# nl1xx/simple-multimodal

Hardware: AMD Instinct MI355X
Metric: fusion fwd+bwd samples/sec at B=16 d=768 (higher is better)
Workload: dtype bf16

## Files before the change

include/mmfusion.h:

```cpp
#ifndef MMFUSION_H
#define MMFUSION_H

#include <stddef.h>
#include <stdint.h>

#ifdef __cplusplus
extern "C" {
#endif

#define MMF_ABI_VERSION 1

enum {
  MMF_OK = 0,
  MMF_E_SHAPE = -1,
  MMF_E_DTYPE = -2,
  MMF_E_ALIGN = -3,
  MMF_E_LAUNCH = -4,
  MMF_E_UNSUPPORTED = -5
};

int mmf_version(void);
const char* mmf_last_error(void);
int mmf_device_cu_count(void);

#define MMF_GEMM_MAX_PROBLEMS 48
enum { MMF_GEMM_NT = 0, MMF_GEMM_NN = 1, MMF_GEMM_TN = 2 };
enum {
  MMF_EPI_BIAS = 1,
  MMF_EPI_RELU = 2,
  MMF_EPI_MASK_AUX = 4,
  MMF_EPI_ADD_AUX = 8,
  MMF_EPI_ACCUM = 16,
  MMF_EPI_COLSUM_A = 32,
  MMF_EPI_DROPOUT = 64
};

typedef struct mmf_gemm_problem {
  const void* A;
  const void* B;
  void* C;
  const float* bias;
  const void* aux;
  int32_t M, N, K;
  int32_t lda, ldb, ldc, ldaux;
} mmf_gemm_problem;

int mmf_gemm_grouped(const mmf_gemm_problem* problems, int num_problems, int layout,
                     int epilogue, int out_f32, void* stream);
typedef struct mmf_gemm_extra {
  float alpha;
  float dropout_p;
  const uint64_t* rng_state;
  uint32_t site;
} mmf_gemm_extra;
int mmf_gemm_grouped_ex(const mmf_gemm_problem* problems, int num_problems, int layout, int epilogue,
                        int out_f32, const mmf_gemm_extra* extra, void* stream);

int mmf_gemm_select_impl(int impl);
int mmf_gemm_last_impl(void);
int mmf_gemm_set_persistent_workgroups(int n);

#define MMF_SKINNY_MAX_PROBLEMS 24
typedef struct mmf_skinny_problem {
  const void* X;
  const void* W;
  void* Y;
  const float* bias;
  const void* aux;
  int32_t M, N, K;
  int32_t ldx, ldw, ldy, ldaux;
} mmf_skinny_problem;
int mmf_skinny_linear_fwd(const mmf_skinny_problem* problems, int num_problems, int flags, int out_f32, void* stream);
int mmf_skinny_linear_dgrad(const mmf_skinny_problem* problems, int num_problems, int flags, float alpha, int out_f32,
                            void* stream);
int mmf_skinny_last_strip(void);
typedef struct mmf_skinny_problem_ex {
  mmf_skinny_problem p;
  void* Y2;
  const void* gate;
  void* dz;
  int32_t ldy2, ldgate, lddz, reserved;
} mmf_skinny_problem_ex;
typedef struct mmf_skinny_extra {
  int32_t x_f32;
  int32_t gate_f32;
  float gate_scale;
  float dropout_p;
  const uint64_t* rng_state;
  uint32_t site;
  uint32_t reserved;
} mmf_skinny_extra;
int mmf_skinny_linear_fwd_ex(const mmf_skinny_problem_ex* problems, int num_problems, int flags, int out_f32,
                             const mmf_skinny_extra* extra, void* stream);
int mmf_skinny_linear_dgrad_ex(const mmf_skinny_problem_ex* problems, int num_problems, int flags, float alpha, int out_f32,
                               const mmf_skinny_extra* extra, void* stream);

int mmf_fusion_loss(const float* logits, int ldl, const int64_t* targets, int B, int C, float label_smoothing,
                    const float* const* extra, const float* extra_w, int n_extra, float* loss, float* dlogits, void* stream);
int mmf_modality_dropout(const float* const* x, float* const* y, float* keep, int B, int d, float p,
                         const uint64_t* rng_state, uint32_t site, int draw, void* stream);

int mmf_distill_kl(const float* student, int lds, const float* teacher, int ldt, int B, int C, float temperature,
                   float* loss, float* dstudent, void* stream);
int mmf_fusion_loss_kd(const float* logits, int ldl, const int64_t* targets, int B, int C, float label_smoothing,
                       const float* const* extra, const float* extra_w, int n_extra,
                       const float* teacher, int ldt, float temperature, float kd_weight,
                       float* loss, float* dlogits, void* stream);

int mmf_robust_head_fwd(const float* const f[3], const float* h, const float* W2, const float* b2,
                        const float* const Wm[3], const float* const bm[3], int avail, float* a, float* const p[3],
                        float* wn, float* y, int B, int d, int C, void* stream);
int mmf_robust_head_bwd(const float* const f[3], const float* h, const float* W2, const float* const Wm[3],
                        const float* a, const float* const p[3], const float* wn, int avail, const float* g,
                        const float* const dP[3], const float* dA, const float* dN, float* const df[3], float* dh,
                        float* dW2, float* db2, float* const dWm[3], float* const dbm[3], int B, int d, int C, void* stream);

int mmf_fewshot_proto_fwd(const float* const s[3], float* sf, float* mean, int n_way, int n_shot, int d, void* stream);
int mmf_fewshot_proto_bwd(const float* dmean, const float* dsf, float* ds, int n_way, int n_shot, int d, void* stream);
int mmf_fewshot_dist_fwd(const float* const q[3], const float* P, float* qf, float* dist, float* pred, int Nq, int n_way,
                         int d, void* stream);
int mmf_fewshot_dist_bwd(const float* qf, const float* P, const float* dist, const float* pred, const float* gdist,
                         const float* gpred, float* dq, float* dp, int Nq, int n_way, int d, void* stream);

#define MMF_EVAL_MAX_HEADS 4
#define MMF_EVAL_NSUMS 4
int mmf_eval_accumulate(const float* const* logits, const int* ld, int n_heads, const int64_t* targets, int B, int C,
                        float label_smoothing, int64_t* counts, double* sums, int64_t* pred_out, int64_t* target_out,
                        float* prob_out, int64_t row0, int64_t capacity, void* stream);

#define MMF_ATTN_MAX_PROBLEMS 12
typedef struct mmf_attn_problem {
  const void* Q; const void* K; const void* V;
  void* O;
  float* LSE;
  const void* dO;
  float* delta;
  void* dQ; void* dK; void* dV;
  int32_t B, H, Tq, Tk;
  int32_t ldq, ldk, ldv, ldo;
} mmf_attn_problem;

int mmf_attn_fwd_grouped(const mmf_attn_problem* problems, int num_problems, int head_dim,
                         float scale, void* stream);
int mmf_attn_bwd_grouped(const mmf_attn_problem* problems, int num_problems, int head_dim,
                         float scale, void* stream);
int mmf_attn_fwd_grouped_ex(const mmf_attn_problem* problems, int num_problems, int head_dim, float scale,
                            float dropout_p, const uint64_t* rng_state, uint32_t site, void* stream);
int mmf_attn_select_impl(int impl);
int mmf_attn_bwd_grouped_ex(const mmf_attn_problem* problems, int num_problems, int head_dim, float scale,
                            float dropout_p, const uint64_t* rng_state, uint32_t site, void* stream);

#define MMF_LN_MAX_PROBLEMS 8
typedef struct mmf_ln_problem {
  const void* x;
  void* y;
  const float* gamma;
  const float* beta;
  float* mean;
  float* rstd;
  const void* dy;
  void* dx;
  float* dgamma;
  float* dbeta;
  int32_t rows;
} mmf_ln_problem;

int mmf_layernorm_fwd_grouped(const mmf_ln_problem* problems, int num_problems, int d, float eps,
                              void* stream);
size_t mmf_layernorm_bwd_workspace_bytes(int d);
int mmf_layernorm_bwd_grouped(const mmf_ln_problem* problems, int num_problems, int d,
                              void* workspace, size_t workspace_bytes, void* stream);
int mmf_layernorm_last_form(void);

int mmf_cast_f32_to_bf16(const float* src, void* dst, int64_t n, void* stream);
int mmf_cast_bf16_to_f32(const void* src, float* dst, int64_t n, void* stream);
int mmf_cast_f32_to_bf16_2d(const float* src, void* dst, int rows, int cols, int ld_src, void* stream);
int mmf_cast_bf16_to_f32_scaled(const void* src, float* dst, int64_t n, float scale, void* stream);
int mmf_add3_bf16(const void* a, const void* b, const void* c, void* y, int64_t n, void* stream);
#define MMF_ADD3_MAX 8
typedef struct mmf_add3_problem {
  const void* a; const void* b; const void* c;
  void* y;
  int64_t n;
} mmf_add3_problem;
int mmf_add3_grouped(const mmf_add3_problem* problems, int num_problems, void* stream);
#define MMF_ADDN_MAX 8
int mmf_addn_bf16(const void* const* xs, int n, void* y, int64_t numel, int out_f32, void* stream);
#define MMF_ADDN_GROUP_MAX 4
typedef struct mmf_addn_problem {
  const void* x[MMF_ADDN_MAX];
  void* y;
  int64_t numel;
  int32_t n;
} mmf_addn_problem;
int mmf_addn_grouped(const mmf_addn_problem* problems, int num_problems, void* stream);
int mmf_meanpool_fwd(const void* x, void* y, int B, int T, int d, int ldy, void* stream);
int mmf_meanpool_bwd(const void* dy, void* dx, int B, int T, int d, int lddy, void* stream);
#define MMF_POOL_MAX 4
int mmf_meanpool_cat_fwd(const void* const* xs, const int* Ts, int n, void* y, int B, int d, int ldy, void* stream);
int mmf_meanpool_cat_bwd(const void* dy, void* const* dxs, const int* Ts, int n, int B, int d, int lddy, void* stream);
int mmf_colsum_bf16(const void* x, float* out, int M, int N, int ldx, void* stream);
#define MMF_COLSUM_MAX_PROBLEMS 24
typedef struct mmf_colsum_problem {
  const void* x;
  float* out;
  int32_t M, N, ldx;
} mmf_colsum_problem;
int mmf_colsum_grouped(const mmf_colsum_problem* problems, int num_problems, void* stream);
int mmf_dropout(const void* x, void* y, int64_t n, int is_f32, float p, const uint64_t* rng_state,
                uint32_t site, void* stream);
#define MMF_ZERO_MAX_RANGES 48
int mmf_zero_ranges_f32(float* base, const int64_t* starts, const int64_t* ends, int n, void* stream);
int mmf_relu_bwd_bf16(const void* dy, const void* y, void* dx, int64_t n, void* stream);
int mmf_relu_bwd_mixed(const void* dy, int dy_f32, const void* y, int y_f32, void* dx, int64_t n, void* stream);

typedef struct mmf_gat3_params {
  int32_t B, heads, C, relu;
  float negative_slope, dropout_p;
  const uint64_t* rng_state;
  uint32_t site;
} mmf_gat3_params;
int mmf_gat3_dense_fwd(const float* h, const float* att_src, const float* att_dst, const float* bias,
                       void* y_bf16, void* pooled_bf16, float* alpha, float* sdots,
                       const mmf_gat3_params* p, void* stream);
int mmf_gat3_dense_bwd(const float* h, const float* att_src, const float* att_dst, const void* y_bf16,
                       const float* alpha, const float* sdots, const void* dy_bf16, const void* dpooled_bf16,
                       float* dh, float* datt_src, float* datt_dst, float* dbias,
                       const mmf_gat3_params* p, void* stream);
int mmf_infonce_fwd(const float* const z[3], float* const n[3], float* inv_norm, float* losses, float* lse,
                    int B, int D, float temperature, void* stream);
int mmf_infonce_bwd(const float* const n[3], const float* inv_norm, const float* lse, const float* const dn[3],
                    const float* const dloss[3], float* const dz[3], int B, int D, float temperature, void* stream);
int mmf_adaptive_combine_fwd(const float* hp, const float* W2, const float* b2, const float* attended,
                             float* aw, void* weighted_bf16, int B, int d, void* stream);
int mmf_adaptive_combine_bwd(const float* hp, const float* W2, const float* attended, const float* aw,
                             const void* dweighted_bf16, const float* daw, float* dattended, float* dhp,
                             float* dW2, float* db2, int B, int d, void* stream);
int mmf_adaptive_attn_weights(const void* qkv_bf16, float* w, int B, int heads, int head_dim, void* stream);
int mmf_attn_weights_mean(const void* qkv_bf16, float* w, int B, int T, int heads, int head_dim, void* stream);
int mmf_linear_narrow_fwd(const float* x, const float* W, const float* b, float* y, int M, int N, int K, void* stream);
int mmf_linear_narrow_bwd(const float* x, const float* W, const float* dy, float* dx, float* dW, float* db,
                          int M, int N, int K, void* stream);
int mmf_stack3_embed_fwd(const float* f0, const float* f1, const float* f2, const float* emb, void* x_bf16,
                         int B, int d, int ldf, void* stream);
int mmf_stack3_embed_bwd(const void* dx_bf16, float* d0, float* d1, float* d2, float* demb, int B, int d, int ldd,
                         void* stream);
int mmf_rowmask_apply(const float* x, const float* mask, float* y, int B, int d, void* stream);

int mmf_sqnorm_f32(const float* x, int64_t n, float* out, void* stream);
int mmf_adamw_advance(int64_t* step, float* hparams, const double* sched, void* stream);
int mmf_adamw_step(float* master, const float* grad, float* exp_avg, float* exp_avg_sq, void* shadow_bf16,
                   int64_t n, const float* hparams, const float* gnorm_sq, void* stream);

int mmf_gemm_f32_grouped(const mmf_gemm_problem* problems, int num_problems, int layout, int epilogue, float alpha,
                         void* stream);
int mmf_gemm_f32_batched(const mmf_gemm_problem* problem, int layout, int epilogue, float alpha, int nb0, int nb1,
                         const int64_t strideA[2], const int64_t strideB[2], const int64_t strideC[2], void* stream);
int mmf_softmax_rows_f32(float* S, int64_t rows, int cols, float scale, void* stream);
int mmf_softmax_bwd_rows_f32(const float* P, float* dP, int64_t rows, int cols, float scale, void* stream);
int mmf_layernorm_f32_fwd(const float* x, float* y, const float* gamma, const float* beta, float* mean, float* rstd,
                          int rows, int d, float eps, void* stream);
int mmf_layernorm_f32_bwd(const float* x, const float* dy, const float* gamma, const float* mean, const float* rstd,
                          float* dx, float* dgamma, float* dbeta, int rows, int d, void* stream);

typedef struct mmf_bilstm_args {
  const void* gx;
  const void* w_hh[2];
  const float* b_ih[2];
  const float* b_hh[2];
  void* y;
  float* gates;
  float* cell;
  const void* dy;
  void* dgates;
  int32_t T, B, H;
} mmf_bilstm_args;
size_t mmf_bilstm_workspace_bytes(void);
int mmf_bilstm_layer_fwd(const mmf_bilstm_args* args, void* workspace, size_t workspace_bytes, void* stream);
int mmf_bilstm_layer_bwd(const mmf_bilstm_args* args, void* workspace, size_t workspace_bytes, void* stream);

int mmf_swap01(const void* in, void* out, int n0, int n1, int d, int in_f32, int out_f32, void* stream);

#ifdef __cplusplus
}
#endif
#endif
```

simple-multimodal_amd/csrc/gemm6.hip:

```cpp
#include "gemm6_parts.h"


#ifndef MMF_G6_DBG
#define MMF_G6_DBG 0
#endif

namespace {

template <bool A_KR, bool B_KR, int BK, int NS, bool OUT_F32>
__device__ __forceinline__ void gemm6_body(const GemmArgs& args, const int total_tiles, char* smem) {
  constexpr int TILE = 256 * BK * 2, STAGE = 2 * TILE, NG = BK / 16, PPO = BK / 8, PPW = 2 * PPO;
  constexpr int WA = A_KR ? 256 : BK, WB = B_KR ? 256 : BK;
  static_assert(NG == 2 || NG == 4, "BK is 32 or 64");

  const int bid = mmf_xcd_tile(blockIdx.x, total_tiles, args.xcd_granule);
  int pi = 0;
  while (pi + 1 < args.nprob && bid >= args.tile_start[pi + 1]) ++pi;
  const mmf_gemm_problem& P = args.p[pi];
  int m0, n0;
  tile_origin(P, bid - args.tile_start[pi], m0, n0);

  const int tid = threadIdx.x, lane = tid & 63;
  const int wave = __builtin_amdgcn_readfirstlane(tid >> 6);
  const int wm = wave >> 1, wn = wave & 1;
  const int M = P.M, N = P.N, K = P.K;
  const int KT = (K + BK - 1) / BK;

  unsigned voff[PPW];
#pragma unroll
  for (int i = 0; i < PPO; ++i) {
    voff[i] = piece_voff<A_KR, BK>(wave + 4 * i, P.lda, lane);
    voff[PPO + i] = piece_voff<B_KR, BK>(wave + 4 * i, P.ldb, lane);
  }
  const unsigned short* Ab = static_cast<const unsigned short*>(P.A) + (A_KR ? (size_t)m0 : (size_t)m0 * P.lda);
  const unsigned short* Bb = static_cast<const unsigned short*>(P.B) + (B_KR ? (size_t)n0 : (size_t)n0 * P.ldb);
  const long recA = A_KR ? ((long)(K - 1) * P.lda + (M - m0)) * 2 : ((long)(M - m0 - 1) * P.lda + K) * 2;
  const long recB = B_KR ? ((long)(K - 1) * P.ldb + (N - n0)) * 2 : ((long)(N - n0 - 1) * P.ldb + K) * 2;
  const int kstepA = A_KR ? BK * P.lda : BK, kstepB = B_KR ? BK * P.ldb : BK;
  char* const my_pieces = smem + wave * 1024;

  auto issue_piece = [&](int kt, int i, bool empty = false) {
    char* st = my_pieces + (kt % NS) * STAGE;
    if (i < PPO) {
      const __amdgpu_buffer_rsrc_t rs = __builtin_amdgcn_make_buffer_rsrc(
          const_cast<unsigned short*>(Ab + (size_t)kt * kstepA), 0, empty ? 0 : (int)(recA - (long)kt * kstepA * 2), 0x00020000);
      __builtin_amdgcn_raw_ptr_buffer_load_lds(rs, (lds_void_t*)(st + i * 4096), 16, voff[i], 0, 0, 0);
    } else {
      const __amdgpu_buffer_rsrc_t rs = __builtin_amdgcn_make_buffer_rsrc(
          const_cast<unsigned short*>(Bb + (size_t)kt * kstepB), 0, empty ? 0 : (int)(recB - (long)kt * kstepB * 2), 0x00020000);
      __builtin_amdgcn_raw_ptr_buffer_load_lds(rs, (lds_void_t*)(st + TILE + (i - PPO) * 4096), 16, voff[i], 0, 0, 0);
    }
  };

  typedef int i32x4_t __attribute__((ext_vector_type(4)));
  auto mkdesc = [](const unsigned short* p, long rec) {
    const unsigned long long a = (unsigned long long)(uintptr_t)p;
    return i32x4_t{(int)(unsigned)a, (int)((unsigned)(a >> 32) & 0xffffu), (int)rec, 0x00020000};
  };
  auto advance = [](i32x4_t& d, int bytes) {
    const unsigned long long a = (((unsigned long long)(unsigned)d[1] << 32) | (unsigned)d[0]) + (unsigned long long)bytes;
    d[0] = (int)(unsigned)a; d[1] = (int)(unsigned)(a >> 32); d[2] -= bytes;
  };
  i32x4_t dA = mkdesc(Ab + (size_t)(NS - 1) * kstepA, recA - (long)(NS - 1) * kstepA * 2);
  i32x4_t dB = mkdesc(Bb + (size_t)(NS - 1) * kstepB, recB - (long)(NS - 1) * kstepB * 2);
  const unsigned lds_pieces = (unsigned)(uintptr_t)(const __attribute__((address_space(3))) char*)my_pieces;
  auto hot_piece = [&](auto ic, const unsigned ring_base) {
    constexpr int I = decltype(ic)::value, OFF = I < PPO ? I * 4096 : TILE + (I - PPO) * 4096;
    if constexpr (MMF_G6_DBG & 16) {
      asm volatile("s_nop 0\n\ts_nop 0\n\ts_nop 0" ::: "memory");
      __builtin_amdgcn_sched_barrier(0);
      return;
    }
    if (I < PPO) asm volatile("s_add_i32 m0, %0, %3\n\ts_nop 0\n\tbuffer_load_dwordx4 %1, %2, 0 offen lds" ::"s"(ring_base), "v"(voff[I]), "s"(dA), "n"(OFF) : "memory");
    else         asm volatile("s_add_i32 m0, %0, %3\n\ts_nop 0\n\tbuffer_load_dwordx4 %1, %2, 0 offen lds" ::"s"(ring_base), "v"(voff[I]), "s"(dB), "n"(OFF) : "memory");
    __builtin_amdgcn_sched_barrier(0);
  };

  unsigned la0, la1, lb0, lb1;
  Frag4<A_KR>::lane_parts(WA, lane, la0, la1);
  Frag4<B_KR>::lane_parts(WB, lane, lb0, lb1);
  const unsigned smem_base = (unsigned)(uintptr_t)(const __attribute__((address_space(3))) char*)smem;
  const unsigned qa = (unsigned)(A_KR ? 512 * 4 * wm : (WA / 32) * 2048 * 4 * wm);
  const unsigned qb = (unsigned)(B_KR ? 512 * 4 * wn : (WB / 32) * 2048 * 4 * wn);
  la0 += smem_base + qa; la1 += smem_base + qa;
  lb0 += smem_base + TILE + qb; lb1 += smem_base + TILE + qb;

  f32x16_t acc[4][4];
  const bool do_colsum = A_KR && (args.epi & MMF_EPI_COLSUM_A) && n0 == 0;
  const bool edge_m = m0 + BM > M;
  bool colok[4];
#pragma unroll
  for (int j = 0; j < 4; ++j) colok[j] = m0 + 128 * wm + 32 * j + (lane & 31) < M;
  f32x16_t csum;
#pragma unroll
  for (int e = 0; e < 16; ++e) csum[e] = 0.f;
  u32x4_t sel[4];
#pragma unroll
  for (int j = 0; j < 4; ++j) {
    const unsigned w = ((lane & 31) == j) ? 0x3f803f80u : 0u;
    sel[j] = u32x4_t{w, w, w, w};
  }

#pragma unroll
  for (int s = 0; s < NS; ++s)
    if (s < KT) {
#pragma unroll
      for (int i = 0; i < PPW; ++i) issue_piece(s, i);
    }
  if (KT >= NS) vm_wait<PPW * (NS - 1)>(); else vm_wait<0>();
  __builtin_amdgcn_s_barrier();
  Frag4<A_KR> fa[2];
  Frag4<B_KR> fb[2];
  fa[0].template issue<WA, 0, 0>(la0, la1);
  fb[0].template issue<WB, 0, 0>(lb0, lb1);
  frag_wait(fa[0], fb[0]);

  auto mf = [&](const Frag4<A_KR>& a, const Frag4<B_KR>& b, int i, bool first = false) {
    const int tm = i >> 2, tn = i & 3;
    const f32x16_t zero = {0.f, 0.f, 0.f, 0.f, 0.f, 0.f, 0.f, 0.f, 0.f, 0.f, 0.f, 0.f, 0.f, 0.f, 0.f, 0.f};
    acc[tn][tm] = __builtin_amdgcn_mfma_f32_32x32x16_bf16(b.get(tn), a.get(tm), first ? zero : acc[tn][tm], 0, 0, 0);
    if (A_KR && do_colsum && tn == 3 && (tm >> 1) == wn) {
      u32x4_t fm = __builtin_bit_cast(u32x4_t, a.get(tm));
      if (edge_m && !colok[tm]) fm = u32x4_t{0u, 0u, 0u, 0u};
      asm volatile("s_nop 1\n\tv_mfma_f32_32x32x16_bf16 %0, %1, %2, %0" : "+v"(csum) : "v"(sel[tm]), "v"(fm));
    }
    __builtin_amdgcn_sched_barrier(0);
  };
#define MMF_G6_READ(dstA, dstB, G, u, so)                                                              \
  do {                                                                                                 \
    if ((u) == 0) dstA.template issue1<WA, G, 0, 0>(la0 + (so), la1 + (so));                            \
    if ((u) == 1) dstA.template issue1<WA, G, 0, 1>(la0 + (so), la1 + (so));                            \
    if ((u) == 2) dstA.template issue1<WA, G, 0, 2>(la0 + (so), la1 + (so));                            \
    if ((u) == 3) dstA.template issue1<WA, G, 0, 3>(la0 + (so), la1 + (so));                            \
    if ((u) == 4) dstB.template issue1<WB, G, 0, 0>(lb0 + (so), lb1 + (so));                            \
    if ((u) == 5) dstB.template issue1<WB, G, 0, 1>(lb0 + (so), lb1 + (so));                            \
    if ((u) == 6) dstB.template issue1<WB, G, 0, 2>(lb0 + (so), lb1 + (so));                            \
    if ((u) == 7) dstB.template issue1<WB, G, 0, 3>(lb0 + (so), lb1 + (so));                            \
    __builtin_amdgcn_sched_barrier(0);                                                                 \
  } while (0)
  static_assert(PPW == 4 + 4 * (NG - 1), "four late pieces + four per not-last substep");
#define MMF_G6_SUBSTEP(cur, nxt, G)                                                                    \
  do {                                                                                                 \
    _Pragma("unroll") for (int i = 0; i < 16; ++i) {                                                   \
      mf(fa[cur], fb[cur], i, FIRST && (G) == 1);                                                      \
      if (i < 8 && !(MMF_G6_DBG & 4)) MMF_G6_READ(fa[nxt], fb[nxt], G, i, so);                        \
      if (i == 8 && !(MMF_G6_DBG & 1)) { if (early) hot_piece(std::integral_constant<int, 4 * (G)>{}, ring_prev); }      \
      if (i == 10 && !(MMF_G6_DBG & 1)) { if (early) hot_piece(std::integral_constant<int, 4 * (G) + 1>{}, ring_prev); } \
      if (i == 12 && !(MMF_G6_DBG & 1)) { if (early) hot_piece(std::integral_constant<int, 4 * (G) + 2>{}, ring_prev); } \
      if (i == 14 && !(MMF_G6_DBG & 1)) { if (early) hot_piece(std::integral_constant<int, 4 * (G) + 3>{}, ring_prev); } \
    }                                                                                                  \
    if (!(MMF_G6_DBG & 4)) frag_wait(fa[nxt], fb[nxt]);                                                \
  } while (0)

  using T = std::true_type;
  using F = std::false_type;
  auto stage = [&](auto next_c, auto steady_c, auto first_c, const int kt, const int ahead, const bool e, const bool l) {
    constexpr bool NEXT = decltype(next_c)::value, STEADY = decltype(steady_c)::value, FIRST = decltype(first_c)::value;
    const bool early = STEADY || e, late = STEADY || l;
    const unsigned so = (unsigned)((kt % NS) * STAGE);
    const unsigned ring_cur = lds_pieces + so, ring_prev = lds_pieces + (unsigned)(((kt + NS - 1) % NS) * STAGE);
    if constexpr (NG == 4) {
      MMF_G6_SUBSTEP(0, 1, 1);
      MMF_G6_SUBSTEP(1, 0, 2);
      MMF_G6_SUBSTEP(0, 1, 3);
    } else {
      MMF_G6_SUBSTEP(0, 1, 1);
    }
    const unsigned sn = (unsigned)(((kt + 1) % NS) * STAGE);
#pragma unroll
    for (int i = 0; i < 4; ++i) mf(fa[1], fb[1], i);
    if constexpr (NEXT) {
      if constexpr (!(MMF_G6_DBG & 2)) {
        if constexpr (STEADY) {
          vm_wait<PPW * (NS - 2)>();
        } else {
          if (ahead >= 3) vm_wait<PPW * 3>(); else if (ahead == 2) vm_wait<PPW * 2>(); else if (ahead == 1) vm_wait<PPW>(); else vm_wait<0>();
        }
        __builtin_amdgcn_s_barrier();
      }
      if constexpr (!(MMF_G6_DBG & 32)) {
        advance(dA, kstepA * 2);
        advance(dB, kstepB * 2);
      }
    }
    __builtin_amdgcn_sched_barrier(0);
#pragma unroll
    for (int i = 4; i < 16; ++i) {
      mf(fa[1], fb[1], i);
      if constexpr (NEXT && !(MMF_G6_DBG & 4)) { if (i < 12) MMF_G6_READ(fa[0], fb[0], 0, i - 4, sn); }
      if (i == 12 && !(MMF_G6_DBG & 1)) { if (late) hot_piece(std::integral_constant<int, 0>{}, ring_cur); }
      if (i == 13 && !(MMF_G6_DBG & 1)) { if (late) hot_piece(std::integral_constant<int, 1>{}, ring_cur); }
      if (i == 14 && !(MMF_G6_DBG & 1)) { if (late) hot_piece(std::integral_constant<int, 2>{}, ring_cur); }
      if (i == 15 && !(MMF_G6_DBG & 1)) { if (late) hot_piece(std::integral_constant<int, 3>{}, ring_cur); }
    }
    if constexpr (NEXT && !(MMF_G6_DBG & 4)) frag_wait(fa[0], fb[0]);
  };
  {
    int kt = 0;
    if (KT > 1) {
      stage(T{}, F{}, T{}, 0, min(NS - 2, KT - 2), false, NS < KT);
      for (kt = 1; kt + NS < KT; ++kt) stage(T{}, T{}, F{}, kt, NS - 2, true, true);
      for (; kt + 1 < KT; ++kt) stage(T{}, F{}, F{}, kt, min(NS - 2, KT - 2 - kt), kt - 1 + NS < KT, kt + NS < KT);
      stage(F{}, F{}, F{}, kt, 0, false, false);
    } else {
      stage(F{}, F{}, T{}, 0, 0, false, false);
    }
  }
#undef MMF_G6_SUBSTEP
#undef MMF_G6_READ

  if (A_KR && do_colsum) {
    asm volatile("s_nop 15\n\ts_nop 7" : "+v"(csum));
    if (lane < 32) {
#pragma unroll
      for (int tm = 0; tm < 4; ++tm) {
        const int m = m0 + 128 * wm + 32 * tm + lane;
        if ((tm >> 1) == wn && m < M) atomicAdd(const_cast<float*>(P.bias) + m, csum[tm]);
      }
    }
  }
  if constexpr (MMF_G6_DBG & 64) {
    float keep = 0.f;
#pragma unroll
    for (int i = 0; i < 4; ++i)
#pragma unroll
      for (int j = 0; j < 4; ++j) keep += acc[i][j][0];
    if (keep == 12345.678f) static_cast<float*>(P.C)[lane] = keep;
    return;
  }
  tile_epilogue<OUT_F32>(args, P, pi, m0 + 128 * wm, n0 + 128 * wn, acc, lane, args.epi);
}

template <bool A_KR, bool B_KR, int BK, int NS, bool OUT_F32>
__global__ __launch_bounds__(NTHREADS, 1)
void gemm6_grouped_kernel(const GemmArgs args, const int total_tiles) {
  __shared__ __attribute__((aligned(1024))) char smem[NS * 2 * 256 * BK * 2];
  gemm6_body<A_KR, B_KR, BK, NS, OUT_F32>(args, total_tiles, smem);
}

template <bool A_KR, bool B_KR, int BK, int NS>
void launch(const GemmArgs& a, int total, int out_f32, hipStream_t s) {
  if (out_f32) hipLaunchKernelGGL((gemm6_grouped_kernel<A_KR, B_KR, BK, NS, true>), dim3(total), dim3(NTHREADS), 0, s, a, total);
  else         hipLaunchKernelGGL((gemm6_grouped_kernel<A_KR, B_KR, BK, NS, false>), dim3(total), dim3(NTHREADS), 0, s, a, total);
}
}

bool mmf_gemm6_supports(const mmf_gemm_problem* problems, int num_problems, int layout) {
  if (layout == MMF_GEMM_TN) return true;
  const int bk = 32;
  for (int i = 0; i < num_problems; ++i)
    if (problems[i].K % bk) return false;
  return true;
}
bool mmf_gemm6_supports_epi(int epilogue, int out_f32) { return !(out_f32 && (epilogue & (MMF_EPI_MASK_AUX | MMF_EPI_ADD_AUX))); }

int mmf_gemm6_launch(const mmf_gemm_problem* problems, int num_problems, int layout, int epilogue,
                     int out_f32, const mmf_gemm_extra* extra, hipStream_t s) {
  GemmArgs a;
  a.nprob = num_problems;
  a.epi = epilogue;
  a.xcd_granule = mmf_xcd_granule();
  a.alpha = extra ? extra->alpha : 1.f;
  a.drop_thresh = extra ? mmf_drop_thresh(extra->dropout_p) : 0u;
  a.site = extra ? extra->site : 0u;
  a.rng_state = extra ? reinterpret_cast<const unsigned long long*>(extra->rng_state) : nullptr;
  int total = 0;
  for (int i = 0; i < num_problems; ++i) {
    const mmf_gemm_problem& p = problems[i];
    const size_t a_bytes = (size_t)(layout == MMF_GEMM_TN ? p.K : p.M) * p.lda * 2;
    const size_t b_bytes = (size_t)(layout == MMF_GEMM_NT ? p.N : p.K) * p.ldb * 2;
    if (a_bytes >= 0x7fffffffull || b_bytes >= 0x7fffffffull)
      MMF_FAIL(MMF_E_UNSUPPORTED, "mmf_gemm_grouped[%d]: operand larger than 2 GiB", i);
    if (layout != MMF_GEMM_TN && p.K % 32)
      MMF_FAIL(MMF_E_UNSUPPORTED, "mmf_gemm_grouped[%d]: the one-wave-per-SIMD kernel needs K %% 32 == 0 for NT / NN (K = %d)", i, p.K);
    if (out_f32 && (epilogue & (MMF_EPI_MASK_AUX | MMF_EPI_ADD_AUX)))
      MMF_FAIL(MMF_E_UNSUPPORTED, "mmf_gemm_grouped: the one-wave-per-SIMD kernel has no aux epilogue with f32 output");
    a.tile_start[i] = total;
    total += ((p.M + BM - 1) / BM) * ((p.N + BN - 1) / BN);
    a.p[i] = p;
  }
  a.tile_start[num_problems] = total;
  static const int cfg = [] { const char* e = getenv("MMF_GEMM6_CFG"); return e ? atoi(e) : 0; }();
  bool k64 = true;
  for (int i = 0; i < num_problems; ++i) k64 = k64 && (problems[i].K % 64 == 0 || layout == MMF_GEMM_TN);
  const int c = (cfg == 2 && !k64) ? 0 : cfg;
  switch (layout) {
    case MMF_GEMM_NT:
      if (c == 1) launch<false, false, 32, 5>(a, total, out_f32, s); else if (c == 2) launch<false, false, 64, 2>(a, total, out_f32, s);
      else launch<false, false, 32, 4>(a, total, out_f32, s);
      break;
    case MMF_GEMM_NN:
      if (c == 1) launch<false, true, 32, 5>(a, total, out_f32, s); else if (c == 2) launch<false, true, 64, 2>(a, total, out_f32, s);
      else launch<false, true, 32, 4>(a, total, out_f32, s);
      break;
    default:
      if (c == 1) launch<true, true, 32, 5>(a, total, out_f32, s); else if (c == 2) launch<true, true, 64, 2>(a, total, out_f32, s);
      else launch<true, true, 32, 4>(a, total, out_f32, s);
      break;
  }
  MMF_CHECK_LAUNCH("mmf_gemm_grouped(v6)");
  return MMF_OK;
}
```

simple-multimodal_amd/csrc/gemm6_parts.h:

```cpp
#pragma once
#include "mmf_internal.h"
#include "lds_image.h"
#include <stdlib.h>
#include <type_traits>

namespace {

constexpr int BM = 256, BN = 256;
constexpr int NTHREADS = 256;

struct GemmArgs {
  int nprob;
  int epi;
  int xcd_granule;
  float alpha;
  unsigned drop_thresh, site;
  const unsigned long long* rng_state;
  int tile_start[MMF_GEMM_MAX_PROBLEMS + 1];
  short orig[MMF_GEMM_MAX_PROBLEMS];
  mmf_gemm_problem p[MMF_GEMM_MAX_PROBLEMS];
};

typedef __attribute__((address_space(3))) void lds_void_t;

template <int N> __device__ __forceinline__ void vm_wait() { asm volatile("s_waitcnt vmcnt(%0)" ::"n"(N) : "memory"); }

template <int OFF>
__device__ __forceinline__ u32x4_t lds_read_b128(unsigned addr) {
  u32x4_t r;
  asm volatile("ds_read_b128 %0, %1 offset:%2" : "=v"(r) : "v"(addr), "n"(OFF));
  return r;
}
template <int OFF>
__device__ __forceinline__ u32x2_t lds_read_tr(unsigned addr) {
  u32x2_t r;
  asm volatile("ds_read_b64_tr_b16 %0, %1 offset:%2" : "=v"(r) : "v"(addr), "n"(OFF));
  return r;
}

template <bool KR> struct Frag4;
template <> struct Frag4<false> {
  u32x4_t v[4];
  static __device__ __forceinline__ void lane_parts(int W, int lane, unsigned& a0, unsigned& a1) {
    const int r = lane & 31, h = lane >> 5, s = (r >> 2) & 3;
    const unsigned base = (unsigned)((W / 32) * 512 * (r >> 3) + 64 * (r & 7));
    a0 = base + 16u * (unsigned)(h ^ s);
    a1 = base + 16u * (unsigned)((2 + h) ^ s);
  }
  template <int W, int G, int D0>
  __device__ __forceinline__ void issue(unsigned t0, unsigned t1) {
    const unsigned t = (G & 1) ? t1 : t0;
    constexpr int S = (W / 32) * 2048;
    v[0] = lds_read_b128<S * (D0 + 0) + 512 * (G >> 1)>(t);
    v[1] = lds_read_b128<S * (D0 + 1) + 512 * (G >> 1)>(t);
    v[2] = lds_read_b128<S * (D0 + 2) + 512 * (G >> 1)>(t);
    v[3] = lds_read_b128<S * (D0 + 3) + 512 * (G >> 1)>(t);
  }
  template <int W, int G, int D0, int I>
  __device__ __forceinline__ void issue1(unsigned t0, unsigned t1) {
    v[I] = lds_read_b128<(W / 32) * 2048 * (D0 + I) + 512 * (G >> 1)>((G & 1) ? t1 : t0);
  }
  __device__ __forceinline__ bf16x8_t get(int i) const { return __builtin_bit_cast(bf16x8_t, v[i]); }
};
template <> struct Frag4<true> {
  u32x2_t lo[4], hi[4];
  static __device__ __forceinline__ void lane_parts(int, int lane, unsigned& a0, unsigned& a1) {
    const int h = lane >> 5, g = (lane >> 4) & 1, q = (lane >> 2) & 3, p = lane & 3;
    const unsigned c = (unsigned)(2 * g + (p >> 1));
    a0 = (unsigned)(4096 * h + 64 * q) + 16u * (c ^ (unsigned)(2 * h)) + 8u * (unsigned)(p & 1);
    a1 = (unsigned)(4096 * h + 64 * (4 + q)) + 16u * (c ^ (unsigned)(2 * h + 1)) + 8u * (unsigned)(p & 1);
  }
  template <int W, int G, int D0>
  __device__ __forceinline__ void issue(unsigned t0, unsigned t1) {
    lo[0] = lds_read_tr<8192 * G + 512 * (D0 + 0)>(t0); hi[0] = lds_read_tr<8192 * G + 512 * (D0 + 0)>(t1);
    lo[1] = lds_read_tr<8192 * G + 512 * (D0 + 1)>(t0); hi[1] = lds_read_tr<8192 * G + 512 * (D0 + 1)>(t1);
    lo[2] = lds_read_tr<8192 * G + 512 * (D0 + 2)>(t0); hi[2] = lds_read_tr<8192 * G + 512 * (D0 + 2)>(t1);
    lo[3] = lds_read_tr<8192 * G + 512 * (D0 + 3)>(t0); hi[3] = lds_read_tr<8192 * G + 512 * (D0 + 3)>(t1);
  }
  template <int W, int G, int D0, int I>
  __device__ __forceinline__ void issue1(unsigned t0, unsigned t1) {
    lo[I] = lds_read_tr<8192 * G + 512 * (D0 + I)>(t0); hi[I] = lds_read_tr<8192 * G + 512 * (D0 + I)>(t1);
  }
  __device__ __forceinline__ bf16x8_t get(int i) const {
    const u32x4_t w = {lo[i][0], lo[i][1], hi[i][0], hi[i][1]};
    return __builtin_bit_cast(bf16x8_t, w);
  }
};
__device__ __forceinline__ void frag_wait(Frag4<false>& a, Frag4<false>& b) {
  asm volatile("s_waitcnt lgkmcnt(0)" : "+v"(a.v[0]), "+v"(a.v[1]), "+v"(a.v[2]), "+v"(a.v[3]), "+v"(b.v[0]), "+v"(b.v[1]), "+v"(b.v[2]), "+v"(b.v[3]));
}
__device__ __forceinline__ void frag_wait(Frag4<false>& a, Frag4<true>& b) {
  asm volatile("s_waitcnt lgkmcnt(0)" : "+v"(a.v[0]), "+v"(a.v[1]), "+v"(a.v[2]), "+v"(a.v[3]), "+v"(b.lo[0]), "+v"(b.lo[1]), "+v"(b.lo[2]), "+v"(b.lo[3]),
               "+v"(b.hi[0]), "+v"(b.hi[1]), "+v"(b.hi[2]), "+v"(b.hi[3]));
}
__device__ __forceinline__ void frag_wait(Frag4<true>& a, Frag4<true>& b) {
  asm volatile("s_waitcnt lgkmcnt(0)" : "+v"(a.lo[0]), "+v"(a.lo[1]), "+v"(a.lo[2]), "+v"(a.lo[3]), "+v"(a.hi[0]), "+v"(a.hi[1]), "+v"(a.hi[2]), "+v"(a.hi[3]),
               "+v"(b.lo[0]), "+v"(b.lo[1]), "+v"(b.lo[2]), "+v"(b.lo[3]), "+v"(b.hi[0]), "+v"(b.hi[1]), "+v"(b.hi[2]), "+v"(b.hi[3]));
}

template <bool KR, int BK>
__device__ __forceinline__ unsigned piece_voff(int p, int ld, int lane) {
  constexpr int NC = (KR ? 256 : BK) / 32;
  const int st = 2 * p + (lane >> 5), rg = st / NC, cc = st % NC;
  const int w = lane & 31, row = 8 * rg + (w >> 2), ch = 4 * cc + ((w & 3) ^ ((row >> 2) & 3));
  return (unsigned)(row * ld * 2 + ch * 16);
}

__device__ __forceinline__ void tile_origin(const mmf_gemm_problem& P, const int t, int& m0, int& n0) {
  const int tiles_m = (P.M + BM - 1) / BM, tiles_n = (P.N + BN - 1) / BN;
#ifdef MMF_GEMM_GROUPM
  constexpr int GROUP_M = MMF_GEMM_GROUPM;
#else
  constexpr int GROUP_M = 8;
#endif
  const int grp = t / (GROUP_M * tiles_n), rem = t % (GROUP_M * tiles_n);
  const int gm = min(GROUP_M, tiles_m - grp * GROUP_M);
  m0 = (grp * GROUP_M + rem % gm) * BM;
  n0 = (rem / gm) * BN;
}

template <bool OUT_F32, int CT>
__device__ __forceinline__ void tile_epilogue_mode(const GemmArgs& args, const mmf_gemm_problem& P, const int pi, const int mb, const int nb,
                                                   f32x16_t (&acc)[4][4], const int lane, const int epi_all) {
  constexpr int MODE = CT < 0 ? 3 : 0;
  const int M = P.M, N = P.N;
  const int epi = CT < 0 ? epi_all : (CT | (epi_all & MMF_EPI_ACCUM));
  const unsigned short* __restrict__ aux = static_cast<const unsigned short*>(P.aux);
  const bool do_drop = MODE == 3 && (epi & MMF_EPI_DROPOUT);
  const unsigned drop_key = do_drop ? mmf_rng_key(*args.rng_state, args.site, (unsigned)pi) : 0u;
  const float drop_scale = do_drop ? 1.f / (1.f - (float)args.drop_thresh * (1.f / 4294967296.f)) : 1.f;
  const float alpha = MODE == 3 ? args.alpha : 1.f;
  const bool use_aux = epi & (MMF_EPI_MASK_AUX | MMF_EPI_ADD_AUX);
  const bool use_old = OUT_F32 && (epi & MMF_EPI_ACCUM);
  const int h = lane >> 5;
  auto ncol = [&](int tn, int g) { return nb + 32 * tn + 8 * g + 4 * h; };

  f32x4_t bv[4][4];
#pragma unroll
  for (int tn = 0; tn < 4; ++tn)
#pragma unroll
    for (int g = 0; g < 4; ++g) {
      bv[tn][g] = f32x4_t{0.f, 0.f, 0.f, 0.f};
      if ((epi & MMF_EPI_BIAS) && ncol(tn, g) < N) bv[tn][g] = *reinterpret_cast<const f32x4_t*>(P.bias + ncol(tn, g));
    }
  auto finish = [&](f32x4_t v, const f32x4_t& b, const u32x2_t& a, int m, int n) -> f32x4_t {
    if constexpr (CT >= 0) {
      if constexpr (CT & MMF_EPI_BIAS) v += b;
      if constexpr (CT & MMF_EPI_RELU) {
#pragma unroll
        for (int e = 0; e < 4; ++e) v[e] = fmaxf(v[e], 0.f);
      }
      if constexpr (CT & (MMF_EPI_MASK_AUX | MMF_EPI_ADD_AUX)) {
        const float a0 = bf16lo(a[0]), a1 = bf16hi(a[0]), a2 = bf16lo(a[1]), a3 = bf16hi(a[1]);
        if constexpr (CT & MMF_EPI_MASK_AUX) {
          v[0] = a0 > 0.f ? v[0] : 0.f; v[1] = a1 > 0.f ? v[1] : 0.f;
          v[2] = a2 > 0.f ? v[2] : 0.f; v[3] = a3 > 0.f ? v[3] : 0.f;
        } else {
          v[0] += a0; v[1] += a1; v[2] += a2; v[3] += a3;
        }
      }
      return v;
    }
    v += b;
    if (epi & MMF_EPI_RELU) {
#pragma unroll
      for (int e = 0; e < 4; ++e) v[e] = fmaxf(v[e], 0.f);
    }
    if (do_drop) {
      const unsigned idx = (unsigned)m * (unsigned)N + (unsigned)n;
#pragma unroll
      for (int e = 0; e < 4; ++e) v[e] = mmf_keep(drop_key, idx + e, args.drop_thresh) ? v[e] * drop_scale : 0.f;
    }
    const float a0 = bf16lo(a[0]), a1 = bf16hi(a[0]), a2 = bf16lo(a[1]), a3 = bf16hi(a[1]);
    if (epi & MMF_EPI_MASK_AUX) {
      v[0] = a0 > 0.f ? v[0] : 0.f; v[1] = a1 > 0.f ? v[1] : 0.f;
      v[2] = a2 > 0.f ? v[2] : 0.f; v[3] = a3 > 0.f ? v[3] : 0.f;
    }
    v *= alpha;
    if (epi & MMF_EPI_ADD_AUX) { v[0] += a0; v[1] += a1; v[2] += a2; v[3] += a3; }
    return v;
  };
  const bool wide = (N & 7) == 0 && (P.ldc & 7) == 0;
  if constexpr (OUT_F32) {
    f32x4_t oldv[2][4];
    auto preload_tile = [&](int t, int slot) {
      const int tm = t >> 2, tn = t & 3, m = mb + 32 * tm + (lane & 31);
#pragma unroll
      for (int g = 0; g < 4; ++g) {
        oldv[slot][g] = f32x4_t{0.f, 0.f, 0.f, 0.f};
        if (m < M && ncol(tn, g) < N)
          oldv[slot][g] = *reinterpret_cast<const f32x4_t*>(static_cast<const float*>(P.C) + (size_t)m * P.ldc + ncol(tn, g));
      }
    };
    if (use_old) preload_tile(0, 0);
#pragma unroll
    for (int t = 0; t < 16; ++t) {
      const int tm = t >> 2, tn = t & 3, m = mb + 32 * tm + (lane & 31);
      f32x4_t v[4];
#pragma unroll
      for (int g = 0; g < 4; ++g) {
        v[g] = f32x4_t{acc[tn][tm][4 * g], acc[tn][tm][4 * g + 1], acc[tn][tm][4 * g + 2], acc[tn][tm][4 * g + 3]};
        v[g] = finish(v[g], bv[tn][g], u32x2_t{0u, 0u}, m, ncol(tn, g));
        if (use_old) v[g] += oldv[t & 1][g];
      }
      if (use_old && t + 1 < 16) preload_tile(t + 1, (t + 1) & 1);
#pragma unroll
      for (int g = 0; g < 4; ++g)
        if (m < M && ncol(tn, g) < N)
          *reinterpret_cast<f32x4_t*>(static_cast<float*>(P.C) + (size_t)m * P.ldc + ncol(tn, g)) = v[g];
    }
  } else {
    u32x2_t axv[2][4];
    auto preload_tile = [&](int t, int slot) {
      const int tm = t >> 2, tn = t & 3, m = mb + 32 * tm + (lane & 31);
#pragma unroll
      for (int g = 0; g < 4; ++g) {
        axv[slot][g] = u32x2_t{0u, 0u};
        if (m < M && ncol(tn, g) < N) axv[slot][g] = *reinterpret_cast<const u32x2_t*>(aux + (size_t)m * P.ldaux + ncol(tn, g));
      }
    };
    if (use_aux) preload_tile(0, 0);
#pragma unroll
    for (int t = 0; t < 16; ++t) {
      const int tm = t >> 2, tn = t & 3, m = mb + 32 * tm + (lane & 31);
      u32x2_t o[4];
#pragma unroll
      for (int g = 0; g < 4; ++g) {
        f32x4_t v = {acc[tn][tm][4 * g], acc[tn][tm][4 * g + 1], acc[tn][tm][4 * g + 2], acc[tn][tm][4 * g + 3]};
        v = finish(v, bv[tn][g], use_aux ? axv[t & 1][g] : u32x2_t{0u, 0u}, m, ncol(tn, g));
        o[g] = u32x2_t{pack_bf16x2(v[0], v[1]), pack_bf16x2(v[2], v[3])};
      }
      if (use_aux && t + 1 < 16) preload_tile(t + 1, (t + 1) & 1);
      if (wide) {
#pragma unroll
        for (int gp = 0; gp < 2; ++gp) {
          const auto r0 = __builtin_amdgcn_permlane32_swap(o[2 * gp][0], o[2 * gp + 1][0], false, false);
          const auto r1 = __builtin_amdgcn_permlane32_swap(o[2 * gp][1], o[2 * gp + 1][1], false, false);
          const u32x4_t w = {r0[0], r1[0], r0[1], r1[1]};
          const int n = nb + 32 * tn + 16 * gp + 8 * h;
          if (m < M && n < N)
            *reinterpret_cast<u32x4_t*>(static_cast<unsigned short*>(P.C) + (size_t)m * P.ldc + n) = w;
        }
      } else {
#pragma unroll
        for (int g = 0; g < 4; ++g)
          if (m < M && ncol(tn, g) < N)
            *reinterpret_cast<u32x2_t*>(static_cast<unsigned short*>(P.C) + (size_t)m * P.ldc + ncol(tn, g)) = o[g];
      }
    }
  }
}

template <bool OUT_F32>
__device__ __forceinline__ void tile_epilogue(const GemmArgs& args, const mmf_gemm_problem& P, const int pi, const int mb, const int nb,
                                              f32x16_t (&acc)[4][4], const int lane, const int epi_all) {
  const int e = epi_all & ~(MMF_EPI_ACCUM | MMF_EPI_COLSUM_A);
  const bool unit = args.alpha == 1.f;
  if (e == 0 && unit)                                              tile_epilogue_mode<OUT_F32, 0>(args, P, pi, mb, nb, acc, lane, epi_all);
  else if (e == MMF_EPI_BIAS && unit)                              tile_epilogue_mode<OUT_F32, MMF_EPI_BIAS>(args, P, pi, mb, nb, acc, lane, epi_all);
  else if (e == (MMF_EPI_BIAS | MMF_EPI_RELU) && unit)             tile_epilogue_mode<OUT_F32, MMF_EPI_BIAS | MMF_EPI_RELU>(args, P, pi, mb, nb, acc, lane, epi_all);
  else if (!OUT_F32 && e == (MMF_EPI_BIAS | MMF_EPI_ADD_AUX) && unit) tile_epilogue_mode<OUT_F32, MMF_EPI_BIAS | MMF_EPI_ADD_AUX>(args, P, pi, mb, nb, acc, lane, epi_all);
  else if (!OUT_F32 && e == MMF_EPI_MASK_AUX && unit)              tile_epilogue_mode<OUT_F32, MMF_EPI_MASK_AUX>(args, P, pi, mb, nb, acc, lane, epi_all);
  else if (!OUT_F32 && e == MMF_EPI_ADD_AUX && unit)               tile_epilogue_mode<OUT_F32, MMF_EPI_ADD_AUX>(args, P, pi, mb, nb, acc, lane, epi_all);
  else                                                             tile_epilogue_mode<OUT_F32, -1>(args, P, pi, mb, nb, acc, lane, epi_all);
}
}
```

simple-multimodal_amd/csrc/gemm7.hip:

```cpp
#include <algorithm>
#include "gemm6_parts.h"

namespace {

constexpr int BK = 32, NS = 4;
constexpr int TILE = 256 * BK * 2, STAGE = 2 * TILE, PPO = BK / 8, PPW = 2 * PPO;

typedef int i32x4_t __attribute__((ext_vector_type(4)));

struct TileSrc {
  const unsigned short* Ab;
  const unsigned short* Bb;
  int recA, recB, stepB, KT;
};
struct TileDst {
  int pi, m0, n0;
};

__device__ __forceinline__ int to_sgpr(int x) {
  int r;
  asm volatile("s_nop 0\n\tv_readfirstlane_b32 %0, %1\n\ts_nop 4" : "=s"(r) : "v"(x));
  return r;
}

template <bool B_KR>
__device__ __forceinline__ void locate_tile(const GemmArgs& args, const int total_tiles, const int orig, TileSrc& s, TileDst& d, int& lda, int& ldb) {
  const int bid = to_sgpr(mmf_xcd_tile(orig, total_tiles, args.xcd_granule));
  int pi = 0;
  while (pi + 1 < args.nprob && bid >= args.tile_start[pi + 1]) ++pi;
  const mmf_gemm_problem& P = args.p[pi];
  int m0, n0;
  tile_origin(P, bid - args.tile_start[pi], m0, n0);
  m0 = to_sgpr(m0);
  n0 = to_sgpr(n0);
  d.pi = pi; d.m0 = m0; d.n0 = n0;
  lda = P.lda; ldb = P.ldb;
  s.Ab = static_cast<const unsigned short*>(P.A) + (size_t)m0 * P.lda;
  s.Bb = static_cast<const unsigned short*>(P.B) + (B_KR ? (size_t)n0 : (size_t)n0 * P.ldb);
  s.recA = (int)(((long)(P.M - m0 - 1) * P.lda + P.K) * 2);
  s.recB = (int)((B_KR ? ((long)(P.K - 1) * P.ldb + (P.N - n0)) : ((long)(P.N - n0 - 1) * P.ldb + P.K)) * 2);
  s.stepB = (B_KR ? BK * P.ldb : BK) * 2;
  s.KT = P.K / BK;
}

template <int CT>
__device__ __forceinline__ void drain_tile(const GemmArgs& args, const int pi, const mmf_gemm_problem& P, const int mb, const int nb,
                                           f32x16_t (&acc)[4][4], char* region, const int lane) {
  constexpr bool AUX = (CT & (MMF_EPI_MASK_AUX | MMF_EPI_ADD_AUX)) != 0;
  constexpr bool DROP = (CT & MMF_EPI_DROPOUT) != 0;
  const unsigned drop_key = DROP ? mmf_rng_key(*args.rng_state, args.site, (unsigned)args.orig[pi]) : 0u;
  const float drop_scale = DROP ? 1.f / (1.f - (float)args.drop_thresh * (1.f / 4294967296.f)) : 1.f;
  const float alpha = (CT & MMF_EPI_MASK_AUX) ? args.alpha : 1.f;
  const int r = lane & 31, h = lane >> 5, q = lane >> 4, cq = lane & 15;
  const unsigned wr_base = (unsigned)(r * 256 + 8 * h + 16 * (r & 15));
  const unsigned rd_base = (unsigned)(q * 256 + ((cq ^ q) << 4));
  auto acc_at = [&](int c) { return region + (wr_base ^ (unsigned)(c << 4)); };
  auto row_at = [&](int it) { return region + it * 1024 + (rd_base ^ (unsigned)((it & 3) << 6)); };
  const bool col_ok = nb + 8 * cq < P.N;
  const __amdgpu_buffer_rsrc_t crs = __builtin_amdgcn_make_buffer_rsrc(P.C, 0, (int)((((long)P.M - 1) * P.ldc + P.N) * 2), 0x00020000);
  const __amdgpu_buffer_rsrc_t ars = __builtin_amdgcn_make_buffer_rsrc(const_cast<void*>(AUX ? P.aux : P.C), 0,
                                                                       AUX ? (int)((((long)P.M - 1) * P.ldaux + P.N) * 2) : 0, 0x00020000);
  const unsigned c_off0 = col_ok ? (unsigned)(((long)(mb + q) * P.ldc + nb + 8 * cq) * 2) : 0x80000000u;
  const unsigned a_off0 = col_ok ? (unsigned)(((long)(mb + q) * P.ldaux + nb + 8 * cq) * 2) : 0x80000000u;
  const unsigned c_row4 = (unsigned)(4 * P.ldc * 2), a_row4 = (unsigned)(4 * P.ldaux * 2);

  u32x4_t auxr[2][8];
  auto load_aux = [&](int tm, int slot) {
#pragma unroll
    for (int it = 0; it < 8; ++it)
      auxr[slot][it] = __builtin_bit_cast(u32x4_t, __builtin_amdgcn_raw_buffer_load_b128(ars, a_off0 + (unsigned)(8 * tm + it) * a_row4, 0, 0));
  };
  if constexpr (AUX) { load_aux(0, 0); load_aux(1, 1); }
#pragma unroll
  for (int tm = 0; tm < 4; ++tm) {
    u32x2_t axv[4][4];
    if constexpr (AUX) {
#pragma unroll
      for (int it = 0; it < 8; ++it) *reinterpret_cast<u32x4_t*>(row_at(it)) = auxr[tm & 1][it];
#pragma unroll
      for (int tn = 0; tn < 4; ++tn)
#pragma unroll
        for (int g = 0; g < 4; ++g) axv[tn][g] = *reinterpret_cast<const u32x2_t*>(acc_at(4 * tn + g));
      __builtin_amdgcn_sched_barrier(0);
      if (tm + 2 < 4) load_aux(tm + 2, tm & 1);
      __builtin_amdgcn_sched_barrier(0);
    }
#pragma unroll
    for (int tn = 0; tn < 4; ++tn) {
      asm volatile("" : "+a"(acc[tn][tm]));
#pragma unroll
      for (int g = 0; g < 4; ++g) {
        f32x4_t v = {acc[tn][tm][4 * g], acc[tn][tm][4 * g + 1], acc[tn][tm][4 * g + 2], acc[tn][tm][4 * g + 3]};
        if constexpr (CT & MMF_EPI_RELU) {
#pragma unroll
          for (int e = 0; e < 4; ++e) v[e] = fmaxf(v[e], 0.f);
        }
        if constexpr (DROP) {
          const unsigned idx = (unsigned)(mb + 32 * tm + r) * (unsigned)P.N + (unsigned)(nb + 32 * tn + 8 * g + 4 * h);
#pragma unroll
          for (int e = 0; e < 4; ++e) v[e] = mmf_keep(drop_key, idx + e, args.drop_thresh) ? v[e] * drop_scale : 0.f;
        }
        if constexpr (AUX) {
          const u32x2_t a = axv[tn][g];
          const float a0 = bf16lo(a[0]), a1 = bf16hi(a[0]), a2 = bf16lo(a[1]), a3 = bf16hi(a[1]);
          if constexpr (CT & MMF_EPI_MASK_AUX) {
            v[0] = a0 > 0.f ? v[0] * alpha : 0.f; v[1] = a1 > 0.f ? v[1] * alpha : 0.f;
            v[2] = a2 > 0.f ? v[2] * alpha : 0.f; v[3] = a3 > 0.f ? v[3] * alpha : 0.f;
          } else {
            v[0] += a0; v[1] += a1; v[2] += a2; v[3] += a3;
          }
        }
        *reinterpret_cast<u32x2_t*>(acc_at(4 * tn + g)) = u32x2_t{pack_bf16x2(v[0], v[1]), pack_bf16x2(v[2], v[3])};
      }
      __builtin_amdgcn_sched_barrier(0);
    }
    u32x4_t w[8];
#pragma unroll
    for (int it = 0; it < 8; ++it) w[it] = *reinterpret_cast<const u32x4_t*>(row_at(it));
#pragma unroll
    for (int it = 0; it < 8; ++it) __builtin_amdgcn_raw_buffer_store_b128(w[it], crs, c_off0 + (unsigned)(8 * tm + it) * c_row4, 0, 0);
    __builtin_amdgcn_sched_barrier(0);
  }
}

template <bool B_KR, int CT>
__device__ __forceinline__ void gemm7_body(const GemmArgs& args, const int total_tiles, char* smem) {
  constexpr bool A_KR = false;
  constexpr int WA = BK, WB = B_KR ? 256 : BK;

  const int tid = threadIdx.x, lane = tid & 63;
  const int wave = __builtin_amdgcn_readfirstlane(tid >> 6);
  const int wm = wave >> 1, wn = wave & 1;
  const int nwg = gridDim.x;
  const int wid = blockIdx.x;
  auto walk = [&](int round) { return round * nwg + ((round & 1) ? nwg - 1 - wid : wid); };
  int round = 0;
  int orig = walk(0);
  TileSrc ns;
  TileDst cd, nd;
  int KT, lda, ldb;
  locate_tile<B_KR>(args, total_tiles, orig, ns, cd, lda, ldb);
  KT = ns.KT;

  unsigned voff[PPW], voffn[PPW];
  auto set_voff = [&](unsigned (&v)[PPW], int la, int lb) {
#pragma unroll
    for (int i = 0; i < PPO; ++i) {
      v[i] = piece_voff<A_KR, BK>(wave + 4 * i, la, lane);
      v[PPO + i] = piece_voff<B_KR, BK>(wave + 4 * i, lb, lane);
    }
  };
  set_voff(voff, lda, ldb);
  char* const my_pieces = smem + wave * 1024;

  struct Desc { int lo, hi, rec; };
  auto mkdesc = [](const unsigned short* p, int rec) {
    const unsigned long long a = (unsigned long long)(uintptr_t)p;
    return Desc{(int)(unsigned)a, (int)((unsigned)(a >> 32) & 0xffffu), rec};
  };
  auto advance = [](Desc& d, int bytes) {
    const unsigned long long a = (((unsigned long long)(unsigned)d.hi << 32) | (unsigned)d.lo) + (unsigned long long)bytes;
    d.lo = (int)(unsigned)a; d.hi = (int)(unsigned)(a >> 32);
    int r;
    asm("s_sub_i32 %0, %1, %2\n\ts_max_i32 %0, %0, 0" : "=s"(r) : "s"(d.rec), "s"(bytes) : "scc");
    d.rec = r;
  };
  Desc dA = mkdesc(ns.Ab, ns.recA);
  Desc dB = mkdesc(ns.Bb, ns.recB);
  constexpr int stepA = BK * 2;
  int stepB = ns.stepB;
  const unsigned lds_pieces = (unsigned)(uintptr_t)(const __attribute__((address_space(3))) char*)my_pieces;
  auto hot_piece = [&](auto ic, const unsigned ring_base) {
    constexpr int I = decltype(ic)::value, OFF = I < PPO ? I * 4096 : TILE + (I - PPO) * 4096;
    const Desc& d = I < PPO ? dA : dB;
    const i32x4_t q = {d.lo, d.hi, d.rec, 0x00020000};
    asm volatile("s_add_i32 m0, %0, %3\n\ts_nop 0\n\tbuffer_load_dwordx4 %1, %2, 0 offen lds" ::"s"(ring_base), "v"(voff[I]), "s"(q), "n"(OFF) : "memory");
    __builtin_amdgcn_sched_barrier(0);
  };

#pragma unroll
  for (int s = 0; s < NS; ++s) {
    const unsigned rb = lds_pieces + (unsigned)(s * STAGE);
    hot_piece(std::integral_constant<int, 0>{}, rb); hot_piece(std::integral_constant<int, 1>{}, rb);
    hot_piece(std::integral_constant<int, 2>{}, rb); hot_piece(std::integral_constant<int, 3>{}, rb);
    if (s + 1 < NS) {
      hot_piece(std::integral_constant<int, 4>{}, rb); hot_piece(std::integral_constant<int, 5>{}, rb);
      hot_piece(std::integral_constant<int, 6>{}, rb); hot_piece(std::integral_constant<int, 7>{}, rb);
      advance(dA, stepA); advance(dB, stepB);
    }
  }

  bool has_next = walk(1) < total_tiles;
  nd = cd;
  if (has_next) {
    int la, lb;
    locate_tile<B_KR>(args, total_tiles, walk(1), ns, nd, la, lb);
    set_voff(voffn, la, lb);
  } else {
    ns.recA = 0; ns.recB = 0; ns.stepB = 0;
#pragma unroll
    for (int i = 0; i < PPW; ++i) voffn[i] = voff[i];
  }

  unsigned la0, la1, lb0, lb1;
  Frag4<A_KR>::lane_parts(WA, lane, la0, la1);
  Frag4<B_KR>::lane_parts(WB, lane, lb0, lb1);
  const unsigned smem_base = (unsigned)(uintptr_t)(const __attribute__((address_space(3))) char*)smem;
  const unsigned qa = (unsigned)((WA / 32) * 2048 * 4 * wm);
  const unsigned qb = (unsigned)(B_KR ? 512 * 4 * wn : (WB / 32) * 2048 * 4 * wn);
  la0 += smem_base + qa; la1 += smem_base + qa;
  lb0 += smem_base + TILE + qb; lb1 += smem_base + TILE + qb;

  f32x16_t acc[4][4];

  constexpr bool use_bias = (CT & MMF_EPI_BIAS) != 0;
  float bcur[4] = {0.f, 0.f, 0.f, 0.f};
  auto load_bias = [&](float (&b)[4], const TileDst& d) {
    const mmf_gemm_problem& P = args.p[d.pi];
    const __amdgpu_buffer_rsrc_t brs = __builtin_amdgcn_make_buffer_rsrc(const_cast<float*>(P.bias), 0, P.N * 4, 0x00020000);
    const unsigned off = (unsigned)((d.n0 + 128 * wn + (lane & 31)) * 4);
#pragma unroll
    for (int tn = 0; tn < 4; ++tn)
      b[tn] = __uint_as_float((unsigned)__builtin_amdgcn_raw_buffer_load_b32(brs, off + (unsigned)(32 * tn * 4), 0, 0));
  };
  auto split3 = [&](float x) {
    const bool lo = lane < 32;
    const unsigned hh = __float_as_uint(x) & 0xffff0000u;
    const float r1 = x - __uint_as_float(hh);
    const unsigned mm = __float_as_uint(r1) & 0xffff0000u;
    const float r2 = r1 - __uint_as_float(mm);
    const unsigned ll = __float_as_uint(r2) & 0xffff0000u;
    const u32x4_t w = {lo ? ((hh >> 16) | mm) : 0u, lo ? (ll >> 16) : 0u, 0u, 0u};
    return __builtin_bit_cast(bf16x8_t, w);
  };
  auto bias_init = [&](const float (&b)[4]) {
    const f32x16_t zero = {0.f, 0.f, 0.f, 0.f, 0.f, 0.f, 0.f, 0.f, 0.f, 0.f, 0.f, 0.f, 0.f, 0.f, 0.f, 0.f};
    const u32x4_t ow = {lane < 32 ? 0x3f803f80u : 0u, lane < 32 ? 0x00003f80u : 0u, 0u, 0u};
    u32x4_t ones[4] = {ow, ow, ow, ow};
#pragma unroll
    for (int tm = 0; tm < 4; ++tm) asm volatile("" : "+v"(ones[tm]));
#pragma unroll
    for (int tn = 0; tn < 4; ++tn) {
      u32x4_t bw = __builtin_bit_cast(u32x4_t, use_bias ? split3(b[tn]) : __builtin_bit_cast(bf16x8_t, u32x4_t{0u, 0u, 0u, 0u}));
      asm volatile("" : "+v"(bw));
#pragma unroll
      for (int tm = 0; tm < 4; ++tm) {
        acc[tn][tm] = __builtin_amdgcn_mfma_f32_32x32x16_bf16(__builtin_bit_cast(bf16x8_t, bw), __builtin_bit_cast(bf16x8_t, ones[tm]), zero, 0, 0, 0);
        __builtin_amdgcn_sched_barrier(0);
      }
    }
  };
  if constexpr (use_bias) load_bias(bcur, cd);

  vm_wait<PPW * (NS - 2) + 4>();
  __builtin_amdgcn_s_barrier();
  Frag4<A_KR> fa[2];
  Frag4<B_KR> fb[2];
  fa[0].template issue<WA, 0, 0>(la0, la1);
  fb[0].template issue<WB, 0, 0>(lb0, lb1);
  frag_wait(fa[0], fb[0]);

  auto mf = [&](const Frag4<A_KR>& a, const Frag4<B_KR>& b, int i) {
    const int tm = i >> 2, tn = i & 3;
    acc[tn][tm] = __builtin_amdgcn_mfma_f32_32x32x16_bf16(b.get(tn), a.get(tm), acc[tn][tm], 0, 0, 0);
    asm volatile("" ::"a"(acc[tn][tm]));
    __builtin_amdgcn_sched_barrier(0);
  };
#define MMF_G7_READ(dstA, dstB, G, u, so)                                                              \
  do {                                                                                                 \
    if ((u) == 0) dstA.template issue1<WA, G, 0, 0>(la0 + (so), la1 + (so));                            \
    if ((u) == 1) dstA.template issue1<WA, G, 0, 1>(la0 + (so), la1 + (so));                            \
    if ((u) == 2) dstA.template issue1<WA, G, 0, 2>(la0 + (so), la1 + (so));                            \
    if ((u) == 3) dstA.template issue1<WA, G, 0, 3>(la0 + (so), la1 + (so));                            \
    if ((u) == 4) dstB.template issue1<WB, G, 0, 0>(lb0 + (so), lb1 + (so));                            \
    if ((u) == 5) dstB.template issue1<WB, G, 0, 1>(lb0 + (so), lb1 + (so));                            \
    if ((u) == 6) dstB.template issue1<WB, G, 0, 2>(lb0 + (so), lb1 + (so));                            \
    if ((u) == 7) dstB.template issue1<WB, G, 0, 3>(lb0 + (so), lb1 + (so));                            \
    __builtin_amdgcn_sched_barrier(0);                                                                 \
  } while (0)

  auto stage = [&](const unsigned g, const int kt, const int ksw) {
    unsigned long long swmask;
    const Desc nA = mkdesc(ns.Ab, ns.recA), nB = mkdesc(ns.Bb, ns.recB);
    const unsigned so = (g % NS) * STAGE;
    const unsigned ring_cur = lds_pieces + so, ring_prev = lds_pieces + ((g + NS - 1) % NS) * STAGE;
#pragma unroll
    for (int i = 0; i < 16; ++i) {
      mf(fa[0], fb[0], i);
      if (i < 8) MMF_G7_READ(fa[1], fb[1], 1, i, so);
      if (i == 8)  hot_piece(std::integral_constant<int, 4>{}, ring_prev);
      if (i == 10) hot_piece(std::integral_constant<int, 5>{}, ring_prev);
      if (i == 12) hot_piece(std::integral_constant<int, 6>{}, ring_prev);
      if (i == 14) hot_piece(std::integral_constant<int, 7>{}, ring_prev);
    }
    frag_wait(fa[1], fb[1]);
    const unsigned sn = ((g + 1) % NS) * STAGE;
#pragma unroll
    for (int i = 0; i < 4; ++i) mf(fa[1], fb[1], i);
    vm_wait<PPW * (NS - 2)>();
    __builtin_amdgcn_s_barrier();
    __builtin_amdgcn_sched_barrier(0);
#pragma unroll
    for (int i = 4; i < 16; ++i) {
      mf(fa[1], fb[1], i);
      if (i < 12) MMF_G7_READ(fa[0], fb[0], 0, i - 4, sn);
      if (i == 4) {
        advance(dA, stepA);
        advance(dB, stepB);
        asm volatile("" ::"s"(dA.lo), "s"(dA.hi), "s"(dA.rec), "s"(dB.lo), "s"(dB.hi), "s"(dB.rec));
        __builtin_amdgcn_sched_barrier(0);
      }
      if (i == 5) {
        asm volatile("s_cmp_eq_u32 %8, %16\n\t"
                     "s_cselect_b32 %0, %9, %0\n\ts_cselect_b32 %1, %10, %1\n\ts_cselect_b32 %2, %11, %2\n\t"
                     "s_cselect_b32 %3, %12, %3\n\ts_cselect_b32 %4, %13, %4\n\ts_cselect_b32 %5, %14, %5\n\t"
                     "s_cselect_b32 %6, %15, %6\n\ts_cselect_b64 %7, -1, 0"
                     : "+s"(dA.lo), "+s"(dA.hi), "+s"(dA.rec), "+s"(dB.lo), "+s"(dB.hi), "+s"(dB.rec), "+s"(stepB), "=s"(swmask)
                     : "s"(kt), "s"(nA.lo), "s"(nA.hi), "s"(nA.rec), "s"(nB.lo), "s"(nB.hi), "s"(nB.rec), "s"(ns.stepB), "s"(ksw)
                     : "scc");
        __builtin_amdgcn_sched_barrier(0);
      }
      if (i == 6) {
        asm volatile("v_cndmask_b32_e64 %0, %0, %4, %8\n\tv_cndmask_b32_e64 %1, %1, %5, %8\n\t"
                     "v_cndmask_b32_e64 %2, %2, %6, %8\n\tv_cndmask_b32_e64 %3, %3, %7, %8"
                     : "+v"(voff[0]), "+v"(voff[1]), "+v"(voff[2]), "+v"(voff[3])
                     : "v"(voffn[0]), "v"(voffn[1]), "v"(voffn[2]), "v"(voffn[3]), "s"(swmask));
        __builtin_amdgcn_sched_barrier(0);
      }
      if (i == 7) {
        asm volatile("v_cndmask_b32_e64 %0, %0, %4, %8\n\tv_cndmask_b32_e64 %1, %1, %5, %8\n\t"
                     "v_cndmask_b32_e64 %2, %2, %6, %8\n\tv_cndmask_b32_e64 %3, %3, %7, %8"
                     : "+v"(voff[4]), "+v"(voff[5]), "+v"(voff[6]), "+v"(voff[7])
                     : "v"(voffn[4]), "v"(voffn[5]), "v"(voffn[6]), "v"(voffn[7]), "s"(swmask));
        __builtin_amdgcn_sched_barrier(0);
      }
      if (i == 12) hot_piece(std::integral_constant<int, 0>{}, ring_cur);
      if (i == 13) hot_piece(std::integral_constant<int, 1>{}, ring_cur);
      if (i == 14) hot_piece(std::integral_constant<int, 2>{}, ring_cur);
      if (i == 15) hot_piece(std::integral_constant<int, 3>{}, ring_cur);
    }
    frag_wait(fa[0], fb[0]);
  };

  char* const region = smem + NS * STAGE + wave * 8192;
  unsigned g = 0;
  for (;;) {
    bias_init(bcur);
    const int ksw = KT - NS;
    for (int kt = 0; kt < KT; ++kt, ++g) stage(g, kt, ksw);
    const mmf_gemm_problem& P = args.p[cd.pi];
    const int mb = cd.m0 + 128 * wm, nb = cd.n0 + 128 * wn;
    if constexpr (use_bias) { if (has_next) load_bias(bcur, nd); }
#ifndef MMF_G7_NODRAIN
    drain_tile<CT & ~MMF_EPI_BIAS>(args, cd.pi, P, mb, nb, acc, region, lane);
#else
    if (lane == 0 && mb == -1) static_cast<volatile unsigned short*>(P.C)[0] = (unsigned short)acc[0][0][0];
#endif
    if (!has_next) break;
    ++round;
    orig = walk(round);
    cd = nd;
    KT = ns.KT;
    has_next = walk(round + 1) < total_tiles;
    if (has_next) {
      int la, lb;
      locate_tile<B_KR>(args, total_tiles, walk(round + 1), ns, nd, la, lb);
      set_voff(voffn, la, lb);
    } else {
      ns.recA = 0; ns.recB = 0; ns.stepB = 0;
    }
  }
  vm_wait<0>();
#undef MMF_G7_READ
}

template <bool B_KR, int CT>
__global__ __launch_bounds__(NTHREADS, 1)
void gemm7_persistent_kernel(const GemmArgs args, const int total_tiles) {
  __shared__ __attribute__((aligned(1024))) char smem[NS * STAGE + 4 * 8192];
  gemm7_body<B_KR, CT>(args, total_tiles, smem);
}

template <bool B_KR, int CT>
void launch7(const GemmArgs& a, int total, int grid, hipStream_t s) {
  hipLaunchKernelGGL((gemm7_persistent_kernel<B_KR, CT>), dim3(grid), dim3(NTHREADS), 0, s, a, total);
}
bool launch7_select(int layout, int eflags, const GemmArgs* a, int total, int grid, hipStream_t s) {
  if (layout == MMF_GEMM_NT) {
    if (eflags == 0)                                      { if (a) launch7<false, 0>(*a, total, grid, s); return true; }
    if (eflags == MMF_EPI_BIAS)                           { if (a) launch7<false, MMF_EPI_BIAS>(*a, total, grid, s); return true; }
    if (eflags == (MMF_EPI_BIAS | MMF_EPI_RELU))          { if (a) launch7<false, MMF_EPI_BIAS | MMF_EPI_RELU>(*a, total, grid, s); return true; }
    if (eflags == (MMF_EPI_BIAS | MMF_EPI_ADD_AUX))       { if (a) launch7<false, MMF_EPI_BIAS | MMF_EPI_ADD_AUX>(*a, total, grid, s); return true; }
    if (eflags == (MMF_EPI_BIAS | MMF_EPI_RELU | MMF_EPI_DROPOUT)) {
      if (a) launch7<false, MMF_EPI_BIAS | MMF_EPI_RELU | MMF_EPI_DROPOUT>(*a, total, grid, s);
      return true;
    }
  } else if (layout == MMF_GEMM_NN) {
    if (eflags == 0)                                      { if (a) launch7<true, 0>(*a, total, grid, s); return true; }
    if (eflags == MMF_EPI_MASK_AUX)                       { if (a) launch7<true, MMF_EPI_MASK_AUX>(*a, total, grid, s); return true; }
    if (eflags == MMF_EPI_ADD_AUX)                        { if (a) launch7<true, MMF_EPI_ADD_AUX>(*a, total, grid, s); return true; }
  }
  return false;
}
}

static int g_persistent_wgs = [] { const char* e = getenv("MMF_GEMM7_WGS"); const int v = e ? atoi(e) : 0; return v > 0 ? v : 0; }();
extern "C" int mmf_gemm_set_persistent_workgroups(int n) {
  if (n < 0 || n > 65536) MMF_FAIL(MMF_E_SHAPE, "mmf_gemm_set_persistent_workgroups: %d not in 0..65536", n);
  g_persistent_wgs = n;
  return MMF_OK;
}

bool mmf_gemm7_supports(const mmf_gemm_problem* problems, int num_problems, int layout, int epilogue, int out_f32, const mmf_gemm_extra* extra) {
  if (out_f32 || !launch7_select(layout, epilogue, nullptr, 0, 0, nullptr)) return false;
  if (extra && extra->alpha != 1.f && !(layout == MMF_GEMM_NN && epilogue == MMF_EPI_MASK_AUX)) return false;
  if ((epilogue & MMF_EPI_DROPOUT) && !(extra && extra->rng_state)) return false;
  for (int i = 0; i < num_problems; ++i) {
    const mmf_gemm_problem& p = problems[i];
    if (p.K % BK || p.K < (NS + 1) * BK || (p.N & 7) || (p.ldc & 7) || (p.aux && (p.ldaux & 7))) return false;
  }
  return true;
}

int mmf_gemm7_launch(const mmf_gemm_problem* problems, int num_problems, int layout, int epilogue,
                     int out_f32, const mmf_gemm_extra* extra, hipStream_t s) {
  if (!mmf_gemm7_supports(problems, num_problems, layout, epilogue, out_f32, extra))
    MMF_FAIL(MMF_E_UNSUPPORTED, "mmf_gemm_grouped: the persistent kernel takes NT / NN launches with bf16 output, K %% 32 == 0, K >= %d, N and the "
             "leading dimensions of C / aux multiples of 8, and the flag sets of the fusion step (alpha only with the NN ReLU mask)", (NS + 1) * BK);
  GemmArgs a;
  a.nprob = num_problems;
  a.epi = epilogue;
  a.xcd_granule = mmf_xcd_granule();
  a.alpha = extra ? extra->alpha : 1.f;
  a.drop_thresh = (extra && (epilogue & MMF_EPI_DROPOUT)) ? mmf_drop_thresh(extra->dropout_p) : 0u;
  a.site = extra ? extra->site : 0u;
  a.rng_state = extra ? reinterpret_cast<const unsigned long long*>(extra->rng_state) : nullptr;
  int total = 0;
  int order[MMF_GEMM_MAX_PROBLEMS];
  for (int i = 0; i < num_problems; ++i) order[i] = i;
  std::stable_sort(order, order + num_problems, [&](int x, int y) { return problems[x].K > problems[y].K; });
  for (int i = 0; i < num_problems; ++i) {
    const mmf_gemm_problem& p = problems[order[i]];
    const size_t a_bytes = (size_t)p.M * p.lda * 2;
    const size_t b_bytes = (size_t)(layout == MMF_GEMM_NT ? p.N : p.K) * p.ldb * 2;
    const size_t c_bytes = (size_t)p.M * p.ldc * 2, x_bytes = p.aux ? (size_t)p.M * p.ldaux * 2 : 0;
    if (a_bytes >= 0x7fffffffull || b_bytes >= 0x7fffffffull || c_bytes >= 0x7fffffffull || x_bytes >= 0x7fffffffull)
      MMF_FAIL(MMF_E_UNSUPPORTED, "mmf_gemm_grouped[%d]: operand larger than 2 GiB", i);
    a.tile_start[i] = total;
    total += ((p.M + BM - 1) / BM) * ((p.N + BN - 1) / BN);
    a.p[i] = p;
    a.orig[i] = (short)order[i];
  }
  a.tile_start[num_problems] = total;
  static const int cus = [] { int c = mmf_device_cu_count(); return c > 0 ? c : 256; }();
  const int want = g_persistent_wgs > 0 ? g_persistent_wgs : cus;
  const int grid = total < want ? total : want;
  launch7_select(layout, epilogue, &a, total, grid, s);
  MMF_CHECK_LAUNCH("mmf_gemm_grouped(v7)");
  return MMF_OK;
}
```

simple-multimodal_amd/csrc/mmf_internal.h:

```cpp
#pragma once
#include <hip/hip_runtime.h>
#include <stdint.h>
#include <stdio.h>
#include <stdlib.h>
#include <stdarg.h>
#include "../../include/mmfusion.h"

typedef __attribute__((ext_vector_type(8))) __bf16 bf16x8_t;
typedef __attribute__((ext_vector_type(4))) short s16x4_t;
typedef __attribute__((ext_vector_type(8))) short s16x8_t;
typedef __attribute__((ext_vector_type(4))) float f32x4_t;
typedef __attribute__((ext_vector_type(16))) float f32x16_t;
typedef __attribute__((ext_vector_type(4))) unsigned u32x4_t;
typedef __attribute__((ext_vector_type(2))) unsigned u32x2_t;

#define MMF_WAVE 64

void mmf_set_error(const char* fmt, ...);
#define MMF_FAIL(code, ...) do { mmf_set_error(__VA_ARGS__); return (code); } while (0)
#define MMF_CHECK_LAUNCH(name) do { hipError_t e_ = hipGetLastError(); \
  if (e_ != hipSuccess) MMF_FAIL(MMF_E_LAUNCH, "%s: launch failed: %s", name, hipGetErrorString(e_)); } while (0)

static inline bool mmf_aligned16(const void* p) { return (reinterpret_cast<uintptr_t>(p) & 15u) == 0; }

__device__ __forceinline__ float bf16_bits_to_f32(unsigned short b) {
  return __uint_as_float(((unsigned)b) << 16);
}
__device__ __forceinline__ unsigned short f32_to_bf16_bits(float f) {
  __bf16 h = (__bf16)f;
  return __builtin_bit_cast(unsigned short, h);
}
__device__ __forceinline__ unsigned pack_bf16x2(float lo, float hi) {
  typedef __attribute__((ext_vector_type(2))) __bf16 bf16x2_t;
  typedef __attribute__((ext_vector_type(2))) float f32x2_t;
  f32x2_t v = {lo, hi};
  bf16x2_t h = __builtin_convertvector(v, bf16x2_t);
  return __builtin_bit_cast(unsigned, h);
}
__device__ __forceinline__ float bf16lo(unsigned w) { return __uint_as_float(w << 16); }
__device__ __forceinline__ float bf16hi(unsigned w) { return __uint_as_float(w & 0xffff0000u); }

__device__ __forceinline__ float wave_sum(float v) {
#pragma unroll
  for (int o = 32; o > 0; o >>= 1) v += __shfl_xor(v, o, 64);
  return v;
}
__device__ __forceinline__ float wave_max(float v) {
#pragma unroll
  for (int o = 32; o > 0; o >>= 1) v = fmaxf(v, __shfl_xor(v, o, 64));
  return v;
}

__device__ __forceinline__ int mmf_xcd_tile(int orig, int total, int G) {
  const int xcd = orig & 7;
  const int full = G > 0 ? (total / (8 * G)) * (8 * G) : 0;
  if (orig < full) {
    const int j = orig >> 3;
    return ((j / G) * 8 + xcd) * G + (j % G);
  }
  const int rest = total - full, q = rest >> 3, r = rest & 7;
  return full + (xcd < r ? xcd * (q + 1) : r * (q + 1) + (xcd - r) * q) + ((orig - full) >> 3);
}
static inline int mmf_xcd_granule() {
  static const int g = [] { const char* e = getenv("MMF_GEMM_XCD_GRANULE"); const int v = e ? atoi(e) : 32; return v > 0 ? v : 0; }();
  return g;
}

__device__ __forceinline__ unsigned mmf_mix32(unsigned x) {
  x ^= x >> 16; x *= 0x7feb352du; x ^= x >> 15; x *= 0x846ca68bu; x ^= x >> 16;
  return x;
}
__device__ __forceinline__ unsigned mmf_rng_key(unsigned long long seed, unsigned site, unsigned sub) {
  return mmf_mix32((unsigned)seed ^ (site * 0x9E3779B9u)) ^ (unsigned)(seed >> 32) ^ (sub * 0x85EBCA6Bu);
}
__device__ __forceinline__ bool mmf_keep(unsigned key, unsigned idx, unsigned thresh) {
  return mmf_mix32(key + idx * 0x9E3779B9u) >= thresh;
}
static inline unsigned mmf_drop_thresh(float p) {
  double t = (double)p * 4294967296.0;
  return t >= 4294967295.0 ? 4294967295u : (unsigned)t;
}

__device__ __forceinline__ s16x4_t lds_read_tr16(const void* lds_addr) {
  return __builtin_amdgcn_ds_read_tr16_b64_v4i16(
      (__attribute__((address_space(3))) s16x4_t*)(lds_addr));
}
```

simple-multimodal_amd/mmfusion/lib.py:

```python
from __future__ import annotations

import ctypes as C
import os
from typing import List, Optional, Sequence

_HERE = os.path.dirname(os.path.abspath(__file__))
LIB_PATH = os.environ.get("MMF_LIB_PATH") or os.path.join(_HERE, "libmmfusion.so")

GEMM_NT, GEMM_NN, GEMM_TN = 0, 1, 2
EPI_BIAS, EPI_RELU, EPI_MASK_AUX, EPI_ADD_AUX, EPI_ACCUM, EPI_COLSUM_A, EPI_DROPOUT = 1, 2, 4, 8, 16, 32, 64
GEMM_MAX_PROBLEMS, ATTN_MAX_PROBLEMS, LN_MAX_PROBLEMS, COLSUM_MAX_PROBLEMS = 48, 12, 8, 24
EVAL_MAX_HEADS, EVAL_NSUMS = 4, 4

SYMBOLS = (
    "mmf_version", "mmf_last_error", "mmf_device_cu_count", "mmf_gemm_grouped", "mmf_gemm_grouped_ex", "mmf_gemm_select_impl", "mmf_gemm_last_impl", "mmf_gemm_set_persistent_workgroups",
    "mmf_attn_fwd_grouped_ex", "mmf_attn_bwd_grouped_ex", "mmf_dropout", "mmf_attn_select_impl",
    "mmf_attn_fwd_grouped", "mmf_attn_bwd_grouped", "mmf_layernorm_fwd_grouped",
    "mmf_layernorm_bwd_grouped", "mmf_layernorm_bwd_workspace_bytes", "mmf_layernorm_last_form", "mmf_cast_f32_to_bf16", "mmf_cast_bf16_to_f32", "mmf_cast_bf16_to_f32_scaled", "mmf_cast_f32_to_bf16_2d", "mmf_add3_bf16", "mmf_add3_grouped", "mmf_addn_bf16", "mmf_addn_grouped",
    "mmf_meanpool_fwd", "mmf_meanpool_bwd", "mmf_meanpool_cat_fwd", "mmf_meanpool_cat_bwd", "mmf_colsum_bf16", "mmf_colsum_grouped", "mmf_relu_bwd_bf16", "mmf_relu_bwd_mixed",
    "mmf_sqnorm_f32", "mmf_adamw_step", "mmf_adamw_advance", "mmf_skinny_linear_fwd", "mmf_skinny_linear_dgrad", "mmf_skinny_linear_fwd_ex", "mmf_skinny_linear_dgrad_ex", "mmf_skinny_last_strip",
    "mmf_gat3_dense_fwd", "mmf_gat3_dense_bwd", "mmf_infonce_fwd", "mmf_infonce_bwd", "mmf_adaptive_combine_fwd",
    "mmf_adaptive_combine_bwd", "mmf_adaptive_attn_weights", "mmf_linear_narrow_fwd", "mmf_linear_narrow_bwd", "mmf_stack3_embed_fwd",
    "mmf_stack3_embed_bwd", "mmf_rowmask_apply", "mmf_zero_ranges_f32", "mmf_fusion_loss", "mmf_modality_dropout",
    "mmf_attn_weights_mean", "mmf_gemm_f32_grouped", "mmf_gemm_f32_batched", "mmf_softmax_rows_f32", "mmf_softmax_bwd_rows_f32",
    "mmf_layernorm_f32_fwd", "mmf_layernorm_f32_bwd", "mmf_bilstm_workspace_bytes", "mmf_bilstm_layer_fwd", "mmf_bilstm_layer_bwd", "mmf_swap01",
    "mmf_distill_kl", "mmf_fusion_loss_kd", "mmf_robust_head_fwd", "mmf_robust_head_bwd",
    "mmf_fewshot_proto_fwd", "mmf_fewshot_proto_bwd", "mmf_fewshot_dist_fwd", "mmf_fewshot_dist_bwd",
    "mmf_eval_accumulate",
)


class GemmProblem(C.Structure):
    _fields_ = [("A", C.c_void_p), ("B", C.c_void_p), ("C", C.c_void_p), ("bias", C.c_void_p),
                ("aux", C.c_void_p), ("M", C.c_int32), ("N", C.c_int32), ("K", C.c_int32),
                ("lda", C.c_int32), ("ldb", C.c_int32), ("ldc", C.c_int32), ("ldaux", C.c_int32)]


class AttnProblem(C.Structure):
    _fields_ = [("Q", C.c_void_p), ("K", C.c_void_p), ("V", C.c_void_p), ("O", C.c_void_p),
                ("LSE", C.c_void_p), ("dO", C.c_void_p), ("delta", C.c_void_p), ("dQ", C.c_void_p),
                ("dK", C.c_void_p), ("dV", C.c_void_p), ("B", C.c_int32), ("H", C.c_int32),
                ("Tq", C.c_int32), ("Tk", C.c_int32), ("ldq", C.c_int32), ("ldk", C.c_int32),
                ("ldv", C.c_int32), ("ldo", C.c_int32)]


class LnProblem(C.Structure):
    _fields_ = [("x", C.c_void_p), ("y", C.c_void_p), ("gamma", C.c_void_p), ("beta", C.c_void_p),
                ("mean", C.c_void_p), ("rstd", C.c_void_p), ("dy", C.c_void_p), ("dx", C.c_void_p),
                ("dgamma", C.c_void_p), ("dbeta", C.c_void_p), ("rows", C.c_int32)]


class GemmExtra(C.Structure):
    _fields_ = [("alpha", C.c_float), ("dropout_p", C.c_float), ("rng_state", C.c_void_p), ("site", C.c_uint32)]


class SkinnyProblem(C.Structure):
    _fields_ = [("X", C.c_void_p), ("W", C.c_void_p), ("Y", C.c_void_p), ("bias", C.c_void_p), ("aux", C.c_void_p),
                ("M", C.c_int32), ("N", C.c_int32), ("K", C.c_int32), ("ldx", C.c_int32), ("ldw", C.c_int32),
                ("ldy", C.c_int32), ("ldaux", C.c_int32)]


class SkinnyProblemEx(C.Structure):
    _fields_ = [("p", SkinnyProblem), ("Y2", C.c_void_p), ("gate", C.c_void_p), ("dz", C.c_void_p),
                ("ldy2", C.c_int32), ("ldgate", C.c_int32), ("lddz", C.c_int32), ("reserved", C.c_int32)]


class SkinnyExtra(C.Structure):
    _fields_ = [("x_f32", C.c_int32), ("gate_f32", C.c_int32), ("gate_scale", C.c_float), ("dropout_p", C.c_float),
                ("rng_state", C.c_void_p), ("site", C.c_uint32), ("reserved", C.c_uint32)]


SKINNY_MAX_M, SKINNY_MAX_PROBLEMS = 64, 24
ADD3_MAX = 8
ADDN_MAX = 8
ADDN_GROUP_MAX = 4


class AddNProblem(C.Structure):
    _fields_ = [("x", C.c_void_p * 8), ("y", C.c_void_p), ("numel", C.c_int64), ("n", C.c_int32)]


class Add3Problem(C.Structure):
    _fields_ = [("a", C.c_void_p), ("b", C.c_void_p), ("c", C.c_void_p), ("y", C.c_void_p), ("n", C.c_int64)]

ZERO_MAX_RANGES = 48
POOL_MAX = 4


class Gat3Params(C.Structure):
    _fields_ = [("B", C.c_int32), ("heads", C.c_int32), ("C", C.c_int32), ("relu", C.c_int32),
                ("negative_slope", C.c_float), ("dropout_p", C.c_float), ("rng_state", C.c_void_p), ("site", C.c_uint32)]


class BiLstmArgs(C.Structure):
    _fields_ = [("gx", C.c_void_p), ("w_hh", C.c_void_p * 2), ("b_ih", C.c_void_p * 2), ("b_hh", C.c_void_p * 2),
                ("y", C.c_void_p), ("gates", C.c_void_p), ("cell", C.c_void_p), ("dy", C.c_void_p), ("dgates", C.c_void_p),
                ("T", C.c_int32), ("B", C.c_int32), ("H", C.c_int32)]


class ColsumProblem(C.Structure):
    _fields_ = [("x", C.c_void_p), ("out", C.c_void_p), ("M", C.c_int32), ("N", C.c_int32), ("ldx", C.c_int32)]


_lib: Optional[C.CDLL] = None


def load() -> C.CDLL:
    global _lib
    if _lib is not None:
        return _lib
    if not os.path.exists(LIB_PATH):
        raise RuntimeError(
            f"{LIB_PATH} is missing: the MI355X fusion path has no fallback. Build it with "
            f"`python -c 'import __graft_entry__ as g; g.build()'` or `make -C simple-multimodal_amd/csrc`.")
    import torch
    lib = C.CDLL(LIB_PATH)
    lib.mmf_last_error.restype = C.c_char_p
    lib.mmf_version.restype = C.c_int
    vp, i32, i64, f32 = C.c_void_p, C.c_int, C.c_int64, C.c_float
    lib.mmf_gemm_grouped.argtypes = [C.POINTER(GemmProblem), i32, i32, i32, i32, vp]
    lib.mmf_gemm_grouped_ex.argtypes = [C.POINTER(GemmProblem), i32, i32, i32, i32, C.POINTER(GemmExtra), vp]
    lib.mmf_attn_fwd_grouped_ex.argtypes = [C.POINTER(AttnProblem), i32, i32, f32, f32, vp, C.c_uint32, vp]
    lib.mmf_attn_bwd_grouped_ex.argtypes = [C.POINTER(AttnProblem), i32, i32, f32, f32, vp, C.c_uint32, vp]
    lib.mmf_dropout.argtypes = [vp, vp, i64, i32, f32, vp, C.c_uint32, vp]
    lib.mmf_attn_fwd_grouped.argtypes = [C.POINTER(AttnProblem), i32, i32, f32, vp]
    lib.mmf_attn_select_impl.argtypes = [i32]
    lib.mmf_attn_bwd_grouped.argtypes = [C.POINTER(AttnProblem), i32, i32, f32, vp]
    lib.mmf_layernorm_fwd_grouped.argtypes = [C.POINTER(LnProblem), i32, i32, f32, vp]
    lib.mmf_layernorm_bwd_grouped.argtypes = [C.POINTER(LnProblem), i32, i32, vp, C.c_size_t, vp]
    lib.mmf_layernorm_bwd_workspace_bytes.argtypes = [i32]
    lib.mmf_layernorm_bwd_workspace_bytes.restype = C.c_size_t
    lib.mmf_cast_f32_to_bf16.argtypes = [vp, vp, i64, vp]
    lib.mmf_cast_bf16_to_f32.argtypes = [vp, vp, i64, vp]
    lib.mmf_cast_bf16_to_f32_scaled.argtypes = [vp, vp, i64, f32, vp]
    lib.mmf_cast_f32_to_bf16_2d.argtypes = [vp, vp, i32, i32, i32, vp]
    lib.mmf_add3_bf16.argtypes = [vp, vp, vp, vp, i64, vp]
    lib.mmf_add3_grouped.argtypes = [C.POINTER(Add3Problem), i32, vp]
    lib.mmf_addn_bf16.argtypes = [C.POINTER(C.c_void_p), i32, vp, i64, i32, vp]
    lib.mmf_addn_grouped.argtypes = [C.POINTER(AddNProblem), i32, vp]
    lib.mmf_meanpool_fwd.argtypes = [vp, vp, i32, i32, i32, i32, vp]
    lib.mmf_meanpool_bwd.argtypes = [vp, vp, i32, i32, i32, i32, vp]
    lib.mmf_meanpool_cat_fwd.argtypes = [C.POINTER(C.c_void_p), C.POINTER(C.c_int), i32, vp, i32, i32, i32, vp]
    lib.mmf_meanpool_cat_bwd.argtypes = [vp, C.POINTER(C.c_void_p), C.POINTER(C.c_int), i32, i32, i32, i32, vp]
    lib.mmf_colsum_bf16.argtypes = [vp, vp, i32, i32, i32, vp]
    lib.mmf_colsum_grouped.argtypes = [C.POINTER(ColsumProblem), i32, vp]
    lib.mmf_relu_bwd_bf16.argtypes = [vp, vp, vp, i64, vp]
    lib.mmf_relu_bwd_mixed.argtypes = [vp, C.c_int, vp, C.c_int, vp, i64, vp]
    lib.mmf_skinny_linear_fwd.argtypes = [C.POINTER(SkinnyProblem), i32, i32, i32, vp]
    lib.mmf_skinny_linear_dgrad.argtypes = [C.POINTER(SkinnyProblem), i32, i32, f32, i32, vp]
    lib.mmf_fusion_loss.argtypes = [vp, i32, vp, i32, i32, f32, C.POINTER(vp), C.POINTER(f32), i32, vp, vp, vp]
    lib.mmf_modality_dropout.argtypes = [C.POINTER(vp), C.POINTER(vp), vp, i32, i32, f32, vp, C.c_uint32, i32, vp]
    lib.mmf_distill_kl.argtypes = [vp, i32, vp, i32, i32, i32, f32, vp, vp, vp]
    lib.mmf_fusion_loss_kd.argtypes = [vp, i32, vp, i32, i32, f32, C.POINTER(vp), C.POINTER(f32), i32, vp, i32, f32, f32, vp, vp, vp]
    pp = C.POINTER(vp)
    lib.mmf_robust_head_fwd.argtypes = [pp, vp, vp, vp, pp, pp, i32, vp, pp, vp, vp, i32, i32, i32, vp]
    lib.mmf_robust_head_bwd.argtypes = [pp, vp, vp, pp, vp, pp, vp, i32, vp, pp, vp, vp, pp, vp, vp, vp, pp, pp,
                                        i32, i32, i32, vp]
    lib.mmf_fewshot_proto_fwd.argtypes = [pp, vp, vp, i32, i32, i32, vp]
    lib.mmf_fewshot_proto_bwd.argtypes = [vp, vp, vp, i32, i32, i32, vp]
    lib.mmf_fewshot_dist_fwd.argtypes = [pp, vp, vp, vp, vp, i32, i32, i32, vp]
    lib.mmf_fewshot_dist_bwd.argtypes = [vp, vp, vp, vp, vp, vp, vp, vp, i32, i32, i32, vp]
    lib.mmf_eval_accumulate.argtypes = [pp, C.POINTER(C.c_int), i32, vp, i32, i32, f32, vp, vp, vp, vp, vp, i64, i64, vp]
    lib.mmf_skinny_linear_fwd_ex.argtypes = [C.POINTER(SkinnyProblemEx), i32, i32, i32, C.POINTER(SkinnyExtra), vp]
    lib.mmf_skinny_linear_dgrad_ex.argtypes = [C.POINTER(SkinnyProblemEx), i32, i32, f32, i32, C.POINTER(SkinnyExtra), vp]
    lib.mmf_sqnorm_f32.argtypes = [vp, i64, vp, vp]
    P3 = C.c_void_p * 3
    lib.mmf_gat3_dense_fwd.argtypes = [vp] * 8 + [C.POINTER(Gat3Params), vp]
    lib.mmf_gat3_dense_bwd.argtypes = [vp] * 12 + [C.POINTER(Gat3Params), vp]
    lib.mmf_infonce_fwd.argtypes = [P3, P3, vp, vp, vp, i32, i32, f32, vp]
    lib.mmf_infonce_bwd.argtypes = [P3, vp, vp, P3, P3, P3, i32, i32, f32, vp]
    lib.mmf_adaptive_combine_fwd.argtypes = [vp] * 6 + [i32, i32, vp]
    lib.mmf_adaptive_combine_bwd.argtypes = [vp] * 10 + [i32, i32, vp]
    lib.mmf_adaptive_attn_weights.argtypes = [vp, vp, i32, i32, i32, vp]
    lib.mmf_attn_weights_mean.argtypes = [vp, vp, i32, i32, i32, i32, vp]
    lib.mmf_linear_narrow_fwd.argtypes = [vp, vp, vp, vp, i32, i32, i32, vp]
    lib.mmf_linear_narrow_bwd.argtypes = [vp, vp, vp, vp, vp, vp, i32, i32, i32, vp]
    lib.mmf_stack3_embed_fwd.argtypes = [vp, vp, vp, vp, vp, i32, i32, i32, vp]
    lib.mmf_stack3_embed_bwd.argtypes = [vp, vp, vp, vp, vp, i32, i32, i32, vp]
    lib.mmf_rowmask_apply.argtypes = [vp, vp, vp, i32, i32, vp]
    lib.mmf_zero_ranges_f32.argtypes = [vp, C.POINTER(C.c_int64), C.POINTER(C.c_int64), i32, vp]
    lib.mmf_adamw_step.argtypes = [vp, vp, vp, vp, vp, i64, vp, vp, vp]
    lib.mmf_adamw_advance.argtypes = [vp, vp, vp, vp]
    lib.mmf_bilstm_workspace_bytes.restype = C.c_size_t
    lib.mmf_bilstm_layer_fwd.argtypes = [C.POINTER(BiLstmArgs), vp, C.c_size_t, vp]
    lib.mmf_bilstm_layer_bwd.argtypes = [C.POINTER(BiLstmArgs), vp, C.c_size_t, vp]
    lib.mmf_swap01.argtypes = [vp, vp, i32, i32, i32, i32, i32, vp]
    S2 = C.c_int64 * 2
    lib.mmf_gemm_f32_grouped.argtypes = [C.POINTER(GemmProblem), i32, i32, i32, f32, vp]
    lib.mmf_gemm_f32_batched.argtypes = [C.POINTER(GemmProblem), i32, i32, f32, i32, i32, S2, S2, S2, vp]
    lib.mmf_softmax_rows_f32.argtypes = [vp, i64, i32, f32, vp]
    lib.mmf_softmax_bwd_rows_f32.argtypes = [vp, vp, i64, i32, f32, vp]
    lib.mmf_layernorm_f32_fwd.argtypes = [vp, vp, vp, vp, vp, vp, i32, i32, f32, vp]
    lib.mmf_layernorm_f32_bwd.argtypes = [vp, vp, vp, vp, vp, vp, vp, vp, i32, i32, vp]
    for name in SYMBOLS:
        getattr(lib, name)
    if lib.mmf_version() != 1:
        raise RuntimeError(f"libmmfusion ABI version {lib.mmf_version()} != 1")
    _lib = lib
    for env, fn in (("MMF_ATTN_IMPL", lib.mmf_attn_select_impl), ("MMF_GEMM_IMPL", lib.mmf_gemm_select_impl)):
        if os.environ.get(env):
            check(fn(int(os.environ[env])))
    return lib


def check(rc: int) -> None:
    if rc != 0:
        raise RuntimeError(f"libmmfusion error {rc}: {load().mmf_last_error().decode()}")


def stream_ptr() -> int:
    import torch
    return torch.cuda.current_stream().cuda_stream


PROFILE: Optional[list] = None
_LAYOUT_NAME = {GEMM_NT: "NT", GEMM_NN: "NN", GEMM_TN: "TN"}


class _Timed:
    def __init__(self, label: str, flops: float, detail=None):
        self.label, self.flops, self.detail = label, flops, detail

    def __enter__(self):
        if PROFILE is not None:
            import torch
            self.e0, self.e1 = torch.cuda.Event(enable_timing=True), torch.cuda.Event(enable_timing=True)
            self.e0.record(torch.cuda.current_stream())
        return self

    def __exit__(self, *exc):
        if PROFILE is not None:
            import torch
            self.e1.record(torch.cuda.current_stream())
            PROFILE.append((self.label, self.flops, self.e0, self.e1, self.detail))


def gemm_grouped(problems: Sequence[GemmProblem], layout: int, epilogue: int, out_f32: bool,
                 alpha: float = 1.0, dropout_p: float = 0.0, rng_state_ptr: Optional[int] = None, site: int = 0) -> None:
    arr = (GemmProblem * len(problems))(*problems)
    flops = sum(2.0 * p.M * p.N * p.K for p in problems) if PROFILE is not None else 0.0
    detail = [(p.M, p.N, p.K) for p in problems] if PROFILE is not None else None
    with _Timed(f"gemm_grouped_kernel<{_LAYOUT_NAME[layout]},{'f32' if out_f32 else 'bf16'}>", flops, detail) as tm:
        if alpha == 1.0 and not (epilogue & EPI_DROPOUT):
            check(load().mmf_gemm_grouped(arr, len(problems), layout, epilogue, int(out_f32), stream_ptr()))
        else:
            ex = GemmExtra(alpha, dropout_p, rng_state_ptr, site)
            check(load().mmf_gemm_grouped_ex(arr, len(problems), layout, epilogue, int(out_f32), C.byref(ex), stream_ptr()))
        if PROFILE is not None:
            tm.label = f"gemm{load().mmf_gemm_last_impl()}_grouped_kernel<{_LAYOUT_NAME[layout]},{'f32' if out_f32 else 'bf16'}>"


def attn_fwd_grouped(problems: Sequence[AttnProblem], head_dim: int, scale: float, dropout_p: float = 0.0,
                     rng_state_ptr: Optional[int] = None, site: int = 0) -> None:
    arr = (AttnProblem * len(problems))(*problems)
    flops = sum(4.0 * p.B * p.H * p.Tq * p.Tk * head_dim for p in problems) if PROFILE is not None else 0.0
    with _Timed(f"attn_fwd_kernel<{head_dim}>", flops, [(p.Tq, p.Tk) for p in problems] if PROFILE is not None else None):
        check(load().mmf_attn_fwd_grouped_ex(arr, len(problems), head_dim, scale, dropout_p, rng_state_ptr, site,
                                             stream_ptr()))


def attn_bwd_grouped(problems: Sequence[AttnProblem], head_dim: int, scale: float, dropout_p: float = 0.0,
                     rng_state_ptr: Optional[int] = None, site: int = 0) -> None:
    arr = (AttnProblem * len(problems))(*problems)
    flops = sum(8.0 * p.B * p.H * p.Tq * p.Tk * head_dim for p in problems) if PROFILE is not None else 0.0
    with _Timed(f"attn_bwd_kernels<{head_dim}>", flops, [(p.Tq, p.Tk) for p in problems] if PROFILE is not None else None):
        check(load().mmf_attn_bwd_grouped_ex(arr, len(problems), head_dim, scale, dropout_p, rng_state_ptr, site,
                                             stream_ptr()))


def layernorm_fwd_grouped(problems: Sequence[LnProblem], d: int, eps: float) -> None:
    arr = (LnProblem * len(problems))(*problems)
    check(load().mmf_layernorm_fwd_grouped(arr, len(problems), d, eps, stream_ptr()))


def layernorm_bwd_grouped(problems: Sequence[LnProblem], d: int, workspace) -> None:
    arr = (LnProblem * len(problems))(*problems)
    check(load().mmf_layernorm_bwd_grouped(arr, len(problems), d, workspace.data_ptr(),
                                           workspace.numel() * workspace.element_size(), stream_ptr()))


def colsum_grouped(problems: Sequence[ColsumProblem]) -> None:
    for i in range(0, len(problems), COLSUM_MAX_PROBLEMS):
        chunk = problems[i:i + COLSUM_MAX_PROBLEMS]
        arr = (ColsumProblem * len(chunk))(*chunk)
        check(load().mmf_colsum_grouped(arr, len(chunk), stream_ptr()))


def skinny_fwd(problems: Sequence[SkinnyProblem], flags: int, out_f32: bool) -> None:
    for i in range(0, len(problems), SKINNY_MAX_PROBLEMS):
        chunk = problems[i:i + SKINNY_MAX_PROBLEMS]
        arr = (SkinnyProblem * len(chunk))(*chunk)
        check(load().mmf_skinny_linear_fwd(arr, len(chunk), flags, int(out_f32), stream_ptr()))


def skinny_fwd_ex(problems: Sequence[SkinnyProblemEx], flags: int, out_f32: bool, extra: SkinnyExtra) -> None:
    if len(problems) > SKINNY_MAX_PROBLEMS:
        raise ValueError("a fused row-linear group must fit one launch")
    arr = (SkinnyProblemEx * len(problems))(*problems)
    check(load().mmf_skinny_linear_fwd_ex(arr, len(problems), flags, int(out_f32), C.byref(extra), stream_ptr()))


def skinny_dgrad_ex(problems: Sequence[SkinnyProblemEx], flags: int, alpha: float, out_f32: bool, extra: SkinnyExtra) -> None:
    if len(problems) > SKINNY_MAX_PROBLEMS:
        raise ValueError("a fused row-linear group must fit one launch")
    arr = (SkinnyProblemEx * len(problems))(*problems)
    check(load().mmf_skinny_linear_dgrad_ex(arr, len(problems), flags, alpha, int(out_f32), C.byref(extra), stream_ptr()))


def skinny_dgrad(problems: Sequence[SkinnyProblem], flags: int, alpha: float, out_f32: bool) -> None:
    for i in range(0, len(problems), SKINNY_MAX_PROBLEMS):
        chunk = problems[i:i + SKINNY_MAX_PROBLEMS]
        arr = (SkinnyProblem * len(chunk))(*chunk)
        check(load().mmf_skinny_linear_dgrad(arr, len(chunk), flags, alpha, int(out_f32), stream_ptr()))
```

Baseline: 7251.

## Add 256x192 tile form to gemm7 chosen by simulated persistent-walk makespan

Templates the persistent gemm7 kernel on the number of N fragments so it can also run 256x192 tiles (three B fragments per wave, less LDS). On the host it simulates the persistent tile walk over the grid and picks the tile width with the smaller max per-workgroup load, caching the choice per shape set. This targets tail imbalance when the tile count does not divide evenly across CUs. The inline asm now declares m0 as an output, and aux alignment is checked. The narrower tile lowers MFMA work per LDS load and adds host-side simulation cost on cache misses.

New measurement: 7433, median of 6. 1.03x the previous value.

```diff
diff --git a/include/mmfusion.h b/include/mmfusion.h
--- a/include/mmfusion.h
+++ b/include/mmfusion.h
@@ -59,6 +59,9 @@
 int mmf_gemm_select_impl(int impl);
 int mmf_gemm_last_impl(void);
 int mmf_gemm_set_persistent_workgroups(int n);
+int mmf_gemm7_set_tile_n(int n);
+int mmf_gemm7_last_tile_n(void);
+int mmf_gemm7_tile_n(const mmf_gemm_problem* problems, int num_problems, int workgroups);
 
 #define MMF_SKINNY_MAX_PROBLEMS 24
 typedef struct mmf_skinny_problem {
diff --git a/simple-multimodal_amd/csrc/gemm6.hip b/simple-multimodal_amd/csrc/gemm6.hip
--- a/simple-multimodal_amd/csrc/gemm6.hip
+++ b/simple-multimodal_amd/csrc/gemm6.hip
@@ -71,8 +71,9 @@
       __builtin_amdgcn_sched_barrier(0);
       return;
     }
-    if (I < PPO) asm volatile("s_add_i32 m0, %0, %3\n\ts_nop 0\n\tbuffer_load_dwordx4 %1, %2, 0 offen lds" ::"s"(ring_base), "v"(voff[I]), "s"(dA), "n"(OFF) : "memory");
-    else         asm volatile("s_add_i32 m0, %0, %3\n\ts_nop 0\n\tbuffer_load_dwordx4 %1, %2, 0 offen lds" ::"s"(ring_base), "v"(voff[I]), "s"(dB), "n"(OFF) : "memory");
+    int m0w;
+    if (I < PPO) asm volatile("s_add_i32 %0, %1, %4\n\ts_nop 0\n\tbuffer_load_dwordx4 %2, %3, 0 offen lds" : "={m0}"(m0w) : "s"(ring_base), "v"(voff[I]), "s"(dA), "n"(OFF) : "memory");
+    else         asm volatile("s_add_i32 %0, %1, %4\n\ts_nop 0\n\tbuffer_load_dwordx4 %2, %3, 0 offen lds" : "={m0}"(m0w) : "s"(ring_base), "v"(voff[I]), "s"(dB), "n"(OFF) : "memory");
     __builtin_amdgcn_sched_barrier(0);
   };
 
diff --git a/simple-multimodal_amd/csrc/gemm6_parts.h b/simple-multimodal_amd/csrc/gemm6_parts.h
--- a/simple-multimodal_amd/csrc/gemm6_parts.h
+++ b/simple-multimodal_amd/csrc/gemm6_parts.h
@@ -38,9 +38,10 @@
   return r;
 }
 
-template <bool KR> struct Frag4;
-template <> struct Frag4<false> {
-  u32x4_t v[4];
+template <bool KR, int NF = 4> struct Frag4;
+template <int NF> struct Frag4<false, NF> {
+  static_assert(NF == 3 || NF == 4, "three or four fragments");
+  u32x4_t v[NF];
   static __device__ __forceinline__ void lane_parts(int W, int lane, unsigned& a0, unsigned& a1) {
     const int r = lane & 31, h = lane >> 5, s = (r >> 2) & 3;
     const unsigned base = (unsigned)((W / 32) * 512 * (r >> 3) + 64 * (r & 7));
@@ -54,7 +55,7 @@
     v[0] = lds_read_b128<S * (D0 + 0) + 512 * (G >> 1)>(t);
     v[1] = lds_read_b128<S * (D0 + 1) + 512 * (G >> 1)>(t);
     v[2] = lds_read_b128<S * (D0 + 2) + 512 * (G >> 1)>(t);
-    v[3] = lds_read_b128<S * (D0 + 3) + 512 * (G >> 1)>(t);
+    if constexpr (NF > 3) v[3] = lds_read_b128<S * (D0 + 3) + 512 * (G >> 1)>(t);
   }
   template <int W, int G, int D0, int I>
   __device__ __forceinline__ void issue1(unsigned t0, unsigned t1) {
@@ -62,24 +63,26 @@
   }
   __device__ __forceinline__ bf16x8_t get(int i) const { return __builtin_bit_cast(bf16x8_t, v[i]); }
 };
-template <> struct Frag4<true> {
-  u32x2_t lo[4], hi[4];
-  static __device__ __forceinline__ void lane_parts(int, int lane, unsigned& a0, unsigned& a1) {
+template <int NF> struct Frag4<true, NF> {
+  static_assert(NF == 3 || NF == 4, "three or four fragments");
+  u32x2_t lo[NF], hi[NF];
+  static __device__ __forceinline__ void lane_parts(int W, int lane, unsigned& a0, unsigned& a1) {
     const int h = lane >> 5, g = (lane >> 4) & 1, q = (lane >> 2) & 3, p = lane & 3;
-    const unsigned c = (unsigned)(2 * g + (p >> 1));
-    a0 = (unsigned)(4096 * h + 64 * q) + 16u * (c ^ (unsigned)(2 * h)) + 8u * (unsigned)(p & 1);
-    a1 = (unsigned)(4096 * h + 64 * (4 + q)) + 16u * (c ^ (unsigned)(2 * h + 1)) + 8u * (unsigned)(p & 1);
+    const unsigned c = (unsigned)(2 * g + (p >> 1)), r8 = (unsigned)((W / 32) * 512);
+    a0 = r8 * (unsigned)h + (unsigned)(64 * q) + 16u * (c ^ (unsigned)(2 * h)) + 8u * (unsigned)(p & 1);
+    a1 = r8 * (unsigned)h + (unsigned)(64 * (4 + q)) + 16u * (c ^ (unsigned)(2 * h + 1)) + 8u * (unsigned)(p & 1);
   }
   template <int W, int G, int D0>
   __device__ __forceinline__ void issue(unsigned t0, unsigned t1) {
-    lo[0] = lds_read_tr<8192 * G + 512 * (D0 + 0)>(t0); hi[0] = lds_read_tr<8192 * G + 512 * (D0 + 0)>(t1);
-    lo[1] = lds_read_tr<8192 * G + 512 * (D0 + 1)>(t0); hi[1] = lds_read_tr<8192 * G + 512 * (D0 + 1)>(t1);
-    lo[2] = lds_read_tr<8192 * G + 512 * (D0 + 2)>(t0); hi[2] = lds_read_tr<8192 * G + 512 * (D0 + 2)>(t1);
-    lo[3] = lds_read_tr<8192 * G + 512 * (D0 + 3)>(t0); hi[3] = lds_read_tr<8192 * G + 512 * (D0 + 3)>(t1);
+    constexpr int R16 = (W / 32) * 1024 * G;
+    lo[0] = lds_read_tr<R16 + 512 * (D0 + 0)>(t0); hi[0] = lds_read_tr<R16 + 512 * (D0 + 0)>(t1);
+    lo[1] = lds_read_tr<R16 + 512 * (D0 + 1)>(t0); hi[1] = lds_read_tr<R16 + 512 * (D0 + 1)>(t1);
+    lo[2] = lds_read_tr<R16 + 512 * (D0 + 2)>(t0); hi[2] = lds_read_tr<R16 + 512 * (D0 + 2)>(t1);
+    if constexpr (NF > 3) { lo[3] = lds_read_tr<R16 + 512 * (D0 + 3)>(t0); hi[3] = lds_read_tr<R16 + 512 * (D0 + 3)>(t1); }
   }
   template <int W, int G, int D0, int I>
   __device__ __forceinline__ void issue1(unsigned t0, unsigned t1) {
-    lo[I] = lds_read_tr<8192 * G + 512 * (D0 + I)>(t0); hi[I] = lds_read_tr<8192 * G + 512 * (D0 + I)>(t1);
+    lo[I] = lds_read_tr<(W / 32) * 1024 * G + 512 * (D0 + I)>(t0); hi[I] = lds_read_tr<(W / 32) * 1024 * G + 512 * (D0 + I)>(t1);
   }
   __device__ __forceinline__ bf16x8_t get(int i) const {
     const u32x4_t w = {lo[i][0], lo[i][1], hi[i][0], hi[i][1]};
@@ -97,17 +100,25 @@
   asm volatile("s_waitcnt lgkmcnt(0)" : "+v"(a.lo[0]), "+v"(a.lo[1]), "+v"(a.lo[2]), "+v"(a.lo[3]), "+v"(a.hi[0]), "+v"(a.hi[1]), "+v"(a.hi[2]), "+v"(a.hi[3]),
                "+v"(b.lo[0]), "+v"(b.lo[1]), "+v"(b.lo[2]), "+v"(b.lo[3]), "+v"(b.hi[0]), "+v"(b.hi[1]), "+v"(b.hi[2]), "+v"(b.hi[3]));
 }
-
-template <bool KR, int BK>
+__device__ __forceinline__ void frag_wait(Frag4<false>& a, Frag4<false, 3>& b) {
+  asm volatile("s_waitcnt lgkmcnt(0)" : "+v"(a.v[0]), "+v"(a.v[1]), "+v"(a.v[2]), "+v"(a.v[3]), "+v"(b.v[0]), "+v"(b.v[1]), "+v"(b.v[2]));
+}
+__device__ __forceinline__ void frag_wait(Frag4<false>& a, Frag4<true, 3>& b) {
+  asm volatile("s_waitcnt lgkmcnt(0)" : "+v"(a.v[0]), "+v"(a.v[1]), "+v"(a.v[2]), "+v"(a.v[3]), "+v"(b.lo[0]), "+v"(b.lo[1]), "+v"(b.lo[2]),
+               "+v"(b.hi[0]), "+v"(b.hi[1]), "+v"(b.hi[2]));
+}
+
+template <bool KR, int BK, int W = 256>
 __device__ __forceinline__ unsigned piece_voff(int p, int ld, int lane) {
-  constexpr int NC = (KR ? 256 : BK) / 32;
+  constexpr int NC = (KR ? W : BK) / 32;
   const int st = 2 * p + (lane >> 5), rg = st / NC, cc = st % NC;
   const int w = lane & 31, row = 8 * rg + (w >> 2), ch = 4 * cc + ((w & 3) ^ ((row >> 2) & 3));
   return (unsigned)(row * ld * 2 + ch * 16);
 }
 
+template <int TBN = BN>
 __device__ __forceinline__ void tile_origin(const mmf_gemm_problem& P, const int t, int& m0, int& n0) {
-  const int tiles_m = (P.M + BM - 1) / BM, tiles_n = (P.N + BN - 1) / BN;
+  const int tiles_m = (P.M + BM - 1) / BM, tiles_n = (P.N + TBN - 1) / TBN;
 #ifdef MMF_GEMM_GROUPM
   constexpr int GROUP_M = MMF_GEMM_GROUPM;
 #else
@@ -116,7 +127,7 @@
   const int grp = t / (GROUP_M * tiles_n), rem = t % (GROUP_M * tiles_n);
   const int gm = min(GROUP_M, tiles_m - grp * GROUP_M);
   m0 = (grp * GROUP_M + rem % gm) * BM;
-  n0 = (rem / gm) * BN;
+  n0 = (rem / gm) * TBN;
 }
 
 template <bool OUT_F32, int CT>
diff --git a/simple-multimodal_amd/csrc/gemm7.hip b/simple-multimodal_amd/csrc/gemm7.hip
--- a/simple-multimodal_amd/csrc/gemm7.hip
+++ b/simple-multimodal_amd/csrc/gemm7.hip
@@ -1,10 +1,16 @@
 #include <algorithm>
+#include <vector>
 #include "gemm6_parts.h"
 
 namespace {
 
 constexpr int BK = 32, NS = 4;
-constexpr int TILE = 256 * BK * 2, STAGE = 2 * TILE, PPO = BK / 8, PPW = 2 * PPO;
+constexpr int TILE = 256 * BK * 2, PPO = BK / 8;
+template <int TN> struct Form {
+  static constexpr int BNT = 64 * TN, TILE_B = BNT * BK * 2, STAGE = TILE + TILE_B, PPB = TN, PPW = PPO + PPB;
+  static constexpr int LDS = NS * STAGE + 4 * 8192;
+};
+static_assert(Form<4>::LDS == 160 * 1024 && Form<3>::LDS == 144 * 1024, "LDS of the two forms");
 
 typedef int i32x4_t __attribute__((ext_vector_type(4)));
 
@@ -23,14 +29,14 @@
   return r;
 }
 
-template <bool B_KR>
+template <bool B_KR, int TN>
 __device__ __forceinline__ void locate_tile(const GemmArgs& args, const int total_tiles, const int orig, TileSrc& s, TileDst& d, int& lda, int& ldb) {
   const int bid = to_sgpr(mmf_xcd_tile(orig, total_tiles, args.xcd_granule));
   int pi = 0;
   while (pi + 1 < args.nprob && bid >= args.tile_start[pi + 1]) ++pi;
   const mmf_gemm_problem& P = args.p[pi];
   int m0, n0;
-  tile_origin(P, bid - args.tile_start[pi], m0, n0);
+  tile_origin<Form<TN>::BNT>(P, bid - args.tile_start[pi], m0, n0);
   m0 = to_sgpr(m0);
   n0 = to_sgpr(n0);
   d.pi = pi; d.m0 = m0; d.n0 = n0;
@@ -43,9 +49,9 @@
   s.KT = P.K / BK;
 }
 
-template <int CT>
+template <int CT, int TN>
 __device__ __forceinline__ void drain_tile(const GemmArgs& args, const int pi, const mmf_gemm_problem& P, const int mb, const int nb,
-                                           f32x16_t (&acc)[4][4], char* region, const int lane) {
+                                           f32x16_t (&acc)[TN][4], char* region, const int lane) {
   constexpr bool AUX = (CT & (MMF_EPI_MASK_AUX | MMF_EPI_ADD_AUX)) != 0;
   constexpr bool DROP = (CT & MMF_EPI_DROPOUT) != 0;
   const unsigned drop_key = DROP ? mmf_rng_key(*args.rng_state, args.site, (unsigned)args.orig[pi]) : 0u;
@@ -56,7 +62,7 @@
   const unsigned rd_base = (unsigned)(q * 256 + ((cq ^ q) << 4));
   auto acc_at = [&](int c) { return region + (wr_base ^ (unsigned)(c << 4)); };
   auto row_at = [&](int it) { return region + it * 1024 + (rd_base ^ (unsigned)((it & 3) << 6)); };
-  const bool col_ok = nb + 8 * cq < P.N;
+  const bool col_ok = cq < 4 * TN && nb + 8 * cq < P.N;
   const __amdgpu_buffer_rsrc_t crs = __builtin_amdgcn_make_buffer_rsrc(P.C, 0, (int)((((long)P.M - 1) * P.ldc + P.N) * 2), 0x00020000);
   const __amdgpu_buffer_rsrc_t ars = __builtin_amdgcn_make_buffer_rsrc(const_cast<void*>(AUX ? P.aux : P.C), 0,
                                                                        AUX ? (int)((((long)P.M - 1) * P.ldaux + P.N) * 2) : 0, 0x00020000);
@@ -73,12 +79,12 @@
   if constexpr (AUX) { load_aux(0, 0); load_aux(1, 1); }
 #pragma unroll
   for (int tm = 0; tm < 4; ++tm) {
-    u32x2_t axv[4][4];
+    u32x2_t axv[TN][4];
     if constexpr (AUX) {
 #pragma unroll
       for (int it = 0; it < 8; ++it) *reinterpret_cast<u32x4_t*>(row_at(it)) = auxr[tm & 1][it];
 #pragma unroll
-      for (int tn = 0; tn < 4; ++tn)
+      for (int tn = 0; tn < TN; ++tn)
 #pragma unroll
         for (int g = 0; g < 4; ++g) axv[tn][g] = *reinterpret_cast<const u32x2_t*>(acc_at(4 * tn + g));
       __builtin_amdgcn_sched_barrier(0);
@@ -86,7 +92,7 @@
       __builtin_amdgcn_sched_barrier(0);
     }
 #pragma unroll
-    for (int tn = 0; tn < 4; ++tn) {
+    for (int tn = 0; tn < TN; ++tn) {
       asm volatile("" : "+a"(acc[tn][tm]));
 #pragma unroll
       for (int g = 0; g < 4; ++g) {
@@ -123,10 +129,12 @@
   }
 }
 
-template <bool B_KR, int CT>
+template <bool B_KR, int CT, int TN>
 __device__ __forceinline__ void gemm7_body(const GemmArgs& args, const int total_tiles, char* smem) {
   constexpr bool A_KR = false;
-  constexpr int WA = BK, WB = B_KR ? 256 : BK;
+  using F = Form<TN>;
+  constexpr int BNT = F::BNT, STAGE = F::STAGE, PPW = F::PPW, NMF = 4 * TN, NRD = 4 + TN;
+  constexpr int WA = BK, WB = B_KR ? BNT : BK;
 
   const int tid = threadIdx.x, lane = tid & 63;
   const int wave = __builtin_amdgcn_readfirstlane(tid >> 6);
@@ -139,16 +147,15 @@
   TileSrc ns;
   TileDst cd, nd;
   int KT, lda, ldb;
-  locate_tile<B_KR>(args, total_tiles, orig, ns, cd, lda, ldb);
+  locate_tile<B_KR, TN>(args, total_tiles, orig, ns, cd, lda, ldb);
   KT = ns.KT;
 
   unsigned voff[PPW], voffn[PPW];
   auto set_voff = [&](unsigned (&v)[PPW], int la, int lb) {
 #pragma unroll
-    for (int i = 0; i < PPO; ++i) {
-      v[i] = piece_voff<A_KR, BK>(wave + 4 * i, la, lane);
-      v[PPO + i] = piece_voff<B_KR, BK>(wave + 4 * i, lb, lane);
-    }
+    for (int i = 0; i < PPO; ++i) v[i] = piece_voff<A_KR, BK>(wave + 4 * i, la, lane);
+#pragma unroll
+    for (int i = 0; i < TN; ++i) v[PPO + i] = piece_voff<B_KR, BK, BNT>(wave + 4 * i, lb, lane);
   };
   set_voff(voff, lda, ldb);
   char* const my_pieces = smem + wave * 1024;
@@ -174,7 +181,8 @@
     constexpr int I = decltype(ic)::value, OFF = I < PPO ? I * 4096 : TILE + (I - PPO) * 4096;
     const Desc& d = I < PPO ? dA : dB;
     const i32x4_t q = {d.lo, d.hi, d.rec, 0x00020000};
-    asm volatile("s_add_i32 m0, %0, %3\n\ts_nop 0\n\tbuffer_load_dwordx4 %1, %2, 0 offen lds" ::"s"(ring_base), "v"(voff[I]), "s"(q), "n"(OFF) : "memory");
+    int m0w;
+    asm volatile("s_add_i32 %0, %1, %4\n\ts_nop 0\n\tbuffer_load_dwordx4 %2, %3, 0 offen lds" : "={m0}"(m0w) : "s"(ring_base), "v"(voff[I]), "s"(q), "n"(OFF) : "memory");
     __builtin_amdgcn_sched_barrier(0);
   };
 
@@ -185,7 +193,8 @@
     hot_piece(std::integral_constant<int, 2>{}, rb); hot_piece(std::integral_constant<int, 3>{}, rb);
     if (s + 1 < NS) {
       hot_piece(std::integral_constant<int, 4>{}, rb); hot_piece(std::integral_constant<int, 5>{}, rb);
-      hot_piece(std::integral_constant<int, 6>{}, rb); hot_piece(std::integral_constant<int, 7>{}, rb);
+      hot_piece(std::integral_constant<int, 6>{}, rb);
+      if constexpr (TN == 4) hot_piece(std::integral_constant<int, 7>{}, rb);
       advance(dA, stepA); advance(dB, stepB);
     }
   }
@@ -194,7 +203,7 @@
   nd = cd;
   if (has_next) {
     int la, lb;
-    locate_tile<B_KR>(args, total_tiles, walk(1), ns, nd, la, lb);
+    locate_tile<B_KR, TN>(args, total_tiles, walk(1), ns, nd, la, lb);
     set_voff(voffn, la, lb);
   } else {
     ns.recA = 0; ns.recB = 0; ns.stepB = 0;
@@ -207,20 +216,20 @@
   Frag4<B_KR>::lane_parts(WB, lane, lb0, lb1);
   const unsigned smem_base = (unsigned)(uintptr_t)(const __attribute__((address_space(3))) char*)smem;
   const unsigned qa = (unsigned)((WA / 32) * 2048 * 4 * wm);
-  const unsigned qb = (unsigned)(B_KR ? 512 * 4 * wn : (WB / 32) * 2048 * 4 * wn);
+  const unsigned qb = (unsigned)(B_KR ? 512 * TN * wn : (WB / 32) * 2048 * TN * wn);
   la0 += smem_base + qa; la1 += smem_base + qa;
   lb0 += smem_base + TILE + qb; lb1 += smem_base + TILE + qb;
 
-  f32x16_t acc[4][4];
+  f32x16_t acc[TN][4];
 
   constexpr bool use_bias = (CT & MMF_EPI_BIAS) != 0;
-  float bcur[4] = {0.f, 0.f, 0.f, 0.f};
-  auto load_bias = [&](float (&b)[4], const TileDst& d) {
+  float bcur[TN] = {};
+  auto load_bias = [&](float (&b)[TN], const TileDst& d) {
     const mmf_gemm_problem& P = args.p[d.pi];
     const __amdgpu_buffer_rsrc_t brs = __builtin_amdgcn_make_buffer_rsrc(const_cast<float*>(P.bias), 0, P.N * 4, 0x00020000);
-    const unsigned off = (unsigned)((d.n0 + 128 * wn + (lane & 31)) * 4);
-#pragma unroll
-    for (int tn = 0; tn < 4; ++tn)
+    const unsigned off = (unsigned)((d.n0 + 32 * TN * wn + (lane & 31)) * 4);
+#pragma unroll
+    for (int tn = 0; tn < TN; ++tn)
       b[tn] = __uint_as_float((unsigned)__builtin_amdgcn_raw_buffer_load_b32(brs, off + (unsigned)(32 * tn * 4), 0, 0));
   };
   auto split3 = [&](float x) {
@@ -233,14 +242,14 @@
     const u32x4_t w = {lo ? ((hh >> 16) | mm) : 0u, lo ? (ll >> 16) : 0u, 0u, 0u};
     return __builtin_bit_cast(bf16x8_t, w);
   };
-  auto bias_init = [&](const float (&b)[4]) {
+  auto bias_init = [&](const float (&b)[TN]) {
     const f32x16_t zero = {0.f, 0.f, 0.f, 0.f, 0.f, 0.f, 0.f, 0.f, 0.f, 0.f, 0.f, 0.f, 0.f, 0.f, 0.f, 0.f};
     const u32x4_t ow = {lane < 32 ? 0x3f803f80u : 0u, lane < 32 ? 0x00003f80u : 0u, 0u, 0u};
     u32x4_t ones[4] = {ow, ow, ow, ow};
 #pragma unroll
     for (int tm = 0; tm < 4; ++tm) asm volatile("" : "+v"(ones[tm]));
 #pragma unroll
-    for (int tn = 0; tn < 4; ++tn) {
+    for (int tn = 0; tn < TN; ++tn) {
       u32x4_t bw = __builtin_bit_cast(u32x4_t, use_bias ? split3(b[tn]) : __builtin_bit_cast(bf16x8_t, u32x4_t{0u, 0u, 0u, 0u}));
       asm volatile("" : "+v"(bw));
 #pragma unroll
@@ -252,16 +261,16 @@
   };
   if constexpr (use_bias) load_bias(bcur, cd);
 
-  vm_wait<PPW * (NS - 2) + 4>();
+  vm_wait<PPW * (NS - 2) + PPO>();
   __builtin_amdgcn_s_barrier();
   Frag4<A_KR> fa[2];
-  Frag4<B_KR> fb[2];
+  Frag4<B_KR, TN> fb[2];
   fa[0].template issue<WA, 0, 0>(la0, la1);
   fb[0].template issue<WB, 0, 0>(lb0, lb1);
   frag_wait(fa[0], fb[0]);
 
-  auto mf = [&](const Frag4<A_KR>& a, const Frag4<B_KR>& b, int i) {
-    const int tm = i >> 2, tn = i & 3;
+  auto mf = [&](const Frag4<A_KR>& a, const Frag4<B_KR, TN>& b, int i) {
+    const int tm = i / TN, tn = i % TN;
     acc[tn][tm] = __builtin_amdgcn_mfma_f32_32x32x16_bf16(b.get(tn), a.get(tm), acc[tn][tm], 0, 0, 0);
     asm volatile("" ::"a"(acc[tn][tm]));
     __builtin_amdgcn_sched_barrier(0);
@@ -275,7 +284,7 @@
     if ((u) == 4) dstB.template issue1<WB, G, 0, 0>(lb0 + (so), lb1 + (so));                            \
     if ((u) == 5) dstB.template issue1<WB, G, 0, 1>(lb0 + (so), lb1 + (so));                            \
     if ((u) == 6) dstB.template issue1<WB, G, 0, 2>(lb0 + (so), lb1 + (so));                            \
-    if ((u) == 7) dstB.template issue1<WB, G, 0, 3>(lb0 + (so), lb1 + (so));                            \
+    if constexpr (TN == 4) { if ((u) == 7) dstB.template issue1<WB, G, 0, TN - 1>(lb0 + (so), lb1 + (so)); } \
     __builtin_amdgcn_sched_barrier(0);                                                                 \
   } while (0)
 
@@ -285,13 +294,13 @@
     const unsigned so = (g % NS) * STAGE;
     const unsigned ring_cur = lds_pieces + so, ring_prev = lds_pieces + ((g + NS - 1) % NS) * STAGE;
 #pragma unroll
-    for (int i = 0; i < 16; ++i) {
+    for (int i = 0; i < NMF; ++i) {
       mf(fa[0], fb[0], i);
-      if (i < 8) MMF_G7_READ(fa[1], fb[1], 1, i, so);
-      if (i == 8)  hot_piece(std::integral_constant<int, 4>{}, ring_prev);
-      if (i == 10) hot_piece(std::integral_constant<int, 5>{}, ring_prev);
-      if (i == 12) hot_piece(std::integral_constant<int, 6>{}, ring_prev);
-      if (i == 14) hot_piece(std::integral_constant<int, 7>{}, ring_prev);
+      if (i < NRD) MMF_G7_READ(fa[1], fb[1], 1, i, so);
+      if (i == NRD)     hot_piece(std::integral_constant<int, 4>{}, ring_prev);
+      if (i == NRD + 2) hot_piece(std::integral_constant<int, 5>{}, ring_prev);
+      if (i == NRD + 4) hot_piece(std::integral_constant<int, 6>{}, ring_prev);
+      if constexpr (TN == 4) { if (i == NRD + 6) hot_piece(std::integral_constant<int, 7>{}, ring_prev); }
     }
     frag_wait(fa[1], fb[1]);
     const unsigned sn = ((g + 1) % NS) * STAGE;
@@ -301,9 +310,9 @@
     __builtin_amdgcn_s_barrier();
     __builtin_amdgcn_sched_barrier(0);
 #pragma unroll
-    for (int i = 4; i < 16; ++i) {
+    for (int i = 4; i < NMF; ++i) {
       mf(fa[1], fb[1], i);
-      if (i < 12) MMF_G7_READ(fa[0], fb[0], 0, i - 4, sn);
+      if (i < 4 + NRD) MMF_G7_READ(fa[0], fb[0], 0, i - 4, sn);
       if (i == 4) {
         advance(dA, stepA);
         advance(dB, stepB);
@@ -328,16 +337,22 @@
         __builtin_amdgcn_sched_barrier(0);
       }
       if (i == 7) {
-        asm volatile("v_cndmask_b32_e64 %0, %0, %4, %8\n\tv_cndmask_b32_e64 %1, %1, %5, %8\n\t"
-                     "v_cndmask_b32_e64 %2, %2, %6, %8\n\tv_cndmask_b32_e64 %3, %3, %7, %8"
-                     : "+v"(voff[4]), "+v"(voff[5]), "+v"(voff[6]), "+v"(voff[7])
-                     : "v"(voffn[4]), "v"(voffn[5]), "v"(voffn[6]), "v"(voffn[7]), "s"(swmask));
+        if constexpr (TN == 4)
+          asm volatile("v_cndmask_b32_e64 %0, %0, %4, %8\n\tv_cndmask_b32_e64 %1, %1, %5, %8\n\t"
+                       "v_cndmask_b32_e64 %2, %2, %6, %8\n\tv_cndmask_b32_e64 %3, %3, %7, %8"
+                       : "+v"(voff[4]), "+v"(voff[5]), "+v"(voff[6]), "+v"(voff[7])
+                       : "v"(voffn[4]), "v"(voffn[5]), "v"(voffn[6]), "v"(voffn[7]), "s"(swmask));
+        else
+          asm volatile("v_cndmask_b32_e64 %0, %0, %3, %6\n\tv_cndmask_b32_e64 %1, %1, %4, %6\n\t"
+                       "v_cndmask_b32_e64 %2, %2, %5, %6"
+                       : "+v"(voff[4]), "+v"(voff[5]), "+v"(voff[6])
+                       : "v"(voffn[4]), "v"(voffn[5]), "v"(voffn[6]), "s"(swmask));
         __builtin_amdgcn_sched_barrier(0);
       }
-      if (i == 12) hot_piece(std::integral_constant<int, 0>{}, ring_cur);
-      if (i == 13) hot_piece(std::integral_constant<int, 1>{}, ring_cur);
-      if (i == 14) hot_piece(std::integral_constant<int, 2>{}, ring_cur);
-      if (i == 15) hot_piece(std::integral_constant<int, 3>{}, ring_cur);
+      if (i == NMF - 4) hot_piece(std::integral_constant<int, 0>{}, ring_cur);
+      if (i == NMF - 3) hot_piece(std::integral_constant<int, 1>{}, ring_cur);
+      if (i == NMF - 2) hot_piece(std::integral_constant<int, 2>{}, ring_cur);
+      if (i == NMF - 1) hot_piece(std::integral_constant<int, 3>{}, ring_cur);
     }
     frag_wait(fa[0], fb[0]);
   };
@@ -349,10 +364,10 @@
     const int ksw = KT - NS;
     for (int kt = 0; kt < KT; ++kt, ++g) stage(g, kt, ksw);
     const mmf_gemm_problem& P = args.p[cd.pi];
-    const int mb = cd.m0 + 128 * wm, nb = cd.n0 + 128 * wn;
+    const int mb = cd.m0 + 128 * wm, nb = cd.n0 + 32 * TN * wn;
     if constexpr (use_bias) { if (has_next) load_bias(bcur, nd); }
 #ifndef MMF_G7_NODRAIN
-    drain_tile<CT & ~MMF_EPI_BIAS>(args, cd.pi, P, mb, nb, acc, region, lane);
+    drain_tile<CT & ~MMF_EPI_BIAS, TN>(args, cd.pi, P, mb, nb, acc, region, lane);
 #else
     if (lane == 0 && mb == -1) static_cast<volatile unsigned short*>(P.C)[0] = (unsigned short)acc[0][0][0];
 #endif
@@ -364,7 +379,7 @@
     has_next = walk(round + 1) < total_tiles;
     if (has_next) {
       int la, lb;
-      locate_tile<B_KR>(args, total_tiles, walk(round + 1), ns, nd, la, lb);
+      locate_tile<B_KR, TN>(args, total_tiles, walk(round + 1), ns, nd, la, lb);
       set_voff(voffn, la, lb);
     } else {
       ns.recA = 0; ns.recB = 0; ns.stepB = 0;
@@ -374,31 +389,32 @@
 #undef MMF_G7_READ
 }
 
-template <bool B_KR, int CT>
+template <bool B_KR, int CT, int TN>
 __global__ __launch_bounds__(NTHREADS, 1)
 void gemm7_persistent_kernel(const GemmArgs args, const int total_tiles) {
-  __shared__ __attribute__((aligned(1024))) char smem[NS * STAGE + 4 * 8192];
-  gemm7_body<B_KR, CT>(args, total_tiles, smem);
+  __shared__ __attribute__((aligned(1024))) char smem[Form<TN>::LDS];
+  gemm7_body<B_KR, CT, TN>(args, total_tiles, smem);
 }
 
 template <bool B_KR, int CT>
-void launch7(const GemmArgs& a, int total, int grid, hipStream_t s) {
-  hipLaunchKernelGGL((gemm7_persistent_kernel<B_KR, CT>), dim3(grid), dim3(NTHREADS), 0, s, a, total);
-}
-bool launch7_select(int layout, int eflags, const GemmArgs* a, int total, int grid, hipStream_t s) {
+void launch7(const GemmArgs& a, int total, int grid, int tile_n, hipStream_t s) {
+  if (tile_n == 192) hipLaunchKernelGGL((gemm7_persistent_kernel<B_KR, CT, 3>), dim3(grid), dim3(NTHREADS), 0, s, a, total);
+  else               hipLaunchKernelGGL((gemm7_persistent_kernel<B_KR, CT, 4>), dim3(grid), dim3(NTHREADS), 0, s, a, total);
+}
+bool launch7_select(int layout, int eflags, const GemmArgs* a, int total, int grid, hipStream_t s, int tile_n = 256) {
   if (layout == MMF_GEMM_NT) {
-    if (eflags == 0)                                      { if (a) launch7<false, 0>(*a, total, grid, s); return true; }
-    if (eflags == MMF_EPI_BIAS)                           { if (a) launch7<false, MMF_EPI_BIAS>(*a, total, grid, s); return true; }
-    if (eflags == (MMF_EPI_BIAS | MMF_EPI_RELU))          { if (a) launch7<false, MMF_EPI_BIAS | MMF_EPI_RELU>(*a, total, grid, s); return true; }
-    if (eflags == (MMF_EPI_BIAS | MMF_EPI_ADD_AUX))       { if (a) launch7<false, MMF_EPI_BIAS | MMF_EPI_ADD_AUX>(*a, total, grid, s); return true; }
+    if (eflags == 0)                                      { if (a) launch7<false, 0>(*a, total, grid, tile_n, s); return true; }
+    if (eflags == MMF_EPI_BIAS)                           { if (a) launch7<false, MMF_EPI_BIAS>(*a, total, grid, tile_n, s); return true; }
+    if (eflags == (MMF_EPI_BIAS | MMF_EPI_RELU))          { if (a) launch7<false, MMF_EPI_BIAS | MMF_EPI_RELU>(*a, total, grid, tile_n, s); return true; }
+    if (eflags == (MMF_EPI_BIAS | MMF_EPI_ADD_AUX))       { if (a) launch7<false, MMF_EPI_BIAS | MMF_EPI_ADD_AUX>(*a, total, grid, tile_n, s); return true; }
     if (eflags == (MMF_EPI_BIAS | MMF_EPI_RELU | MMF_EPI_DROPOUT)) {
-      if (a) launch7<false, MMF_EPI_BIAS | MMF_EPI_RELU | MMF_EPI_DROPOUT>(*a, total, grid, s);
+      if (a) launch7<false, MMF_EPI_BIAS | MMF_EPI_RELU | MMF_EPI_DROPOUT>(*a, total, grid, tile_n, s);
       return true;
     }
   } else if (layout == MMF_GEMM_NN) {
-    if (eflags == 0)                                      { if (a) launch7<true, 0>(*a, total, grid, s); return true; }
-    if (eflags == MMF_EPI_MASK_AUX)                       { if (a) launch7<true, MMF_EPI_MASK_AUX>(*a, total, grid, s); return true; }
-    if (eflags == MMF_EPI_ADD_AUX)                        { if (a) launch7<true, MMF_EPI_ADD_AUX>(*a, total, grid, s); return true; }
+    if (eflags == 0)                                      { if (a) launch7<true, 0>(*a, total, grid, tile_n, s); return true; }
+    if (eflags == MMF_EPI_MASK_AUX)                       { if (a) launch7<true, MMF_EPI_MASK_AUX>(*a, total, grid, tile_n, s); return true; }
+    if (eflags == MMF_EPI_ADD_AUX)                        { if (a) launch7<true, MMF_EPI_ADD_AUX>(*a, total, grid, tile_n, s); return true; }
   }
   return false;
 }
@@ -409,6 +425,74 @@
   if (n < 0 || n > 65536) MMF_FAIL(MMF_E_SHAPE, "mmf_gemm_set_persistent_workgroups: %d not in 0..65536", n);
   g_persistent_wgs = n;
   return MMF_OK;
+}
+static int g_tile_n = 0;
+static thread_local int t_last_tile_n = 0;
+extern "C" int mmf_gemm7_set_tile_n(int n) {
+  if (n != 0 && n != 256 && n != 192) MMF_FAIL(MMF_E_SHAPE, "mmf_gemm7_set_tile_n: %d is not 0, 256 or 192", n);
+  g_tile_n = n;
+  return MMF_OK;
+}
+extern "C" int mmf_gemm7_last_tile_n(void) { return t_last_tile_n; }
+
+namespace {
+int persistent_grid_cap() {
+  static const int cus = [] { int c = mmf_device_cu_count(); return c > 0 ? c : 256; }();
+  return g_persistent_wgs > 0 ? g_persistent_wgs : cus;
+}
+int tiles_of(const mmf_gemm_problem& p, int bn) { return ((p.M + BM - 1) / BM) * ((p.N + bn - 1) / bn); }
+long long walk_makespan(const mmf_gemm_problem* problems, const int* order, int n, int bn, int cap, int granule) {
+  int start[MMF_GEMM_MAX_PROBLEMS + 1];
+  start[0] = 0;
+  for (int i = 0; i < n; ++i) start[i + 1] = start[i] + tiles_of(problems[order[i]], bn);
+  const int total = start[n], grid = total < cap ? total : cap;
+  if (total == 0) return 0;
+  static thread_local std::vector<long long> load;
+  load.assign(grid, 0);
+  for (int o = 0; o < total; ++o) {
+    const int round = o / grid, pos = o % grid, wid = (round & 1) ? grid - 1 - pos : pos;
+    const int bid = mmf_xcd_tile(o, total, granule);
+    const int pi = (int)(std::upper_bound(start, start + n + 1, bid) - start) - 1;
+    load[wid] += (long long)problems[order[pi]].K * bn;
+  }
+  return *std::max_element(load.begin(), load.end());
+}
+struct TileNMemo {
+  int cap, granule, n, width;
+  int mnk[3 * MMF_GEMM_MAX_PROBLEMS];
+};
+int pick_tile_n(const mmf_gemm_problem* problems, const int* order, int n, int cap) {
+  const int granule = mmf_xcd_granule();
+  static thread_local TileNMemo memo[16];
+  static thread_local int used = 0, next = 0;
+  TileNMemo key;
+  key.cap = cap; key.granule = granule; key.n = n;
+  for (int i = 0; i < n; ++i) {
+    const mmf_gemm_problem& p = problems[order[i]];
+    key.mnk[3 * i] = p.M; key.mnk[3 * i + 1] = p.N; key.mnk[3 * i + 2] = p.K;
+  }
+  for (int e = 0; e < used; ++e) {
+    const TileNMemo& m = memo[e];
+    if (m.cap == cap && m.granule == granule && m.n == n && std::equal(key.mnk, key.mnk + 3 * n, m.mnk)) return m.width;
+  }
+  key.width = walk_makespan(problems, order, n, 192, cap, granule) < walk_makespan(problems, order, n, 256, cap, granule) ? 192 : 256;
+  memo[next] = key;
+  next = (next + 1) % 16;
+  if (used < 16) ++used;
+  return key.width;
+}
+void sort_by_k(const mmf_gemm_problem* problems, int n, int* order) {
+  for (int i = 0; i < n; ++i) order[i] = i;
+  std::stable_sort(order, order + n, [&](int x, int y) { return problems[x].K > problems[y].K; });
+}
+}
+
+extern "C" int mmf_gemm7_tile_n(const mmf_gemm_problem* problems, int num_problems, int workgroups) {
+  if (!problems || num_problems < 1 || num_problems > MMF_GEMM_MAX_PROBLEMS || workgroups < 0)
+    MMF_FAIL(MMF_E_SHAPE, "mmf_gemm7_tile_n: %d problems, %d workgroups", num_problems, workgroups);
+  int order[MMF_GEMM_MAX_PROBLEMS];
+  sort_by_k(problems, num_problems, order);
+  return pick_tile_n(problems, order, num_problems, workgroups > 0 ? workgroups : persistent_grid_cap());
 }
 
 bool mmf_gemm7_supports(const mmf_gemm_problem* problems, int num_problems, int layout, int epilogue, int out_f32, const mmf_gemm_extra* extra) {
@@ -417,7 +501,7 @@
   if ((epilogue & MMF_EPI_DROPOUT) && !(extra && extra->rng_state)) return false;
   for (int i = 0; i < num_problems; ++i) {
     const mmf_gemm_problem& p = problems[i];
-    if (p.K % BK || p.K < (NS + 1) * BK || (p.N & 7) || (p.ldc & 7) || (p.aux && (p.ldaux & 7))) return false;
+    if (p.K % BK || p.K < (NS + 1) * BK || (p.N & 7) || (p.ldc & 7) || (p.aux && ((p.ldaux & 7) || !mmf_aligned16(p.aux)))) return false;
   }
   return true;
 }
@@ -437,8 +521,9 @@
   a.rng_state = extra ? reinterpret_cast<const unsigned long long*>(extra->rng_state) : nullptr;
   int total = 0;
   int order[MMF_GEMM_MAX_PROBLEMS];
-  for (int i = 0; i < num_problems; ++i) order[i] = i;
-  std::stable_sort(order, order + num_problems, [&](int x, int y) { return problems[x].K > problems[y].K; });
+  sort_by_k(problems, num_problems, order);
+  const int cap = persistent_grid_cap();
+  const int tile_n = g_tile_n ? g_tile_n : pick_tile_n(problems, order, num_problems, cap);
   for (int i = 0; i < num_problems; ++i) {
     const mmf_gemm_problem& p = problems[order[i]];
     const size_t a_bytes = (size_t)p.M * p.lda * 2;
@@ -447,15 +532,14 @@
     if (a_bytes >= 0x7fffffffull || b_bytes >= 0x7fffffffull || c_bytes >= 0x7fffffffull || x_bytes >= 0x7fffffffull)
       MMF_FAIL(MMF_E_UNSUPPORTED, "mmf_gemm_grouped[%d]: operand larger than 2 GiB", i);
     a.tile_start[i] = total;
-    total += ((p.M + BM - 1) / BM) * ((p.N + BN - 1) / BN);
+    total += tiles_of(p, tile_n);
     a.p[i] = p;
     a.orig[i] = (short)order[i];
   }
   a.tile_start[num_problems] = total;
-  static const int cus = [] { int c = mmf_device_cu_count(); return c > 0 ? c : 256; }();
-  const int want = g_persistent_wgs > 0 ? g_persistent_wgs : cus;
-  const int grid = total < want ? total : want;
-  launch7_select(layout, epilogue, &a, total, grid, s);
+  const int grid = total < cap ? total : cap;
+  t_last_tile_n = tile_n;
+  launch7_select(layout, epilogue, &a, total, grid, s, tile_n);
   MMF_CHECK_LAUNCH("mmf_gemm_grouped(v7)");
   return MMF_OK;
 }
diff --git a/simple-multimodal_amd/csrc/mmf_internal.h b/simple-multimodal_amd/csrc/mmf_internal.h
--- a/simple-multimodal_amd/csrc/mmf_internal.h
+++ b/simple-multimodal_amd/csrc/mmf_internal.h
@@ -51,7 +51,7 @@
   return v;
 }
 
-__device__ __forceinline__ int mmf_xcd_tile(int orig, int total, int G) {
+__host__ __device__ __forceinline__ int mmf_xcd_tile(int orig, int total, int G) {
   const int xcd = orig & 7;
   const int full = G > 0 ? (total / (8 * G)) * (8 * G) : 0;
   if (orig < full) {
diff --git a/simple-multimodal_amd/mmfusion/lib.py b/simple-multimodal_amd/mmfusion/lib.py
--- a/simple-multimodal_amd/mmfusion/lib.py
+++ b/simple-multimodal_amd/mmfusion/lib.py
@@ -14,6 +14,7 @@
 
 SYMBOLS = (
     "mmf_version", "mmf_last_error", "mmf_device_cu_count", "mmf_gemm_grouped", "mmf_gemm_grouped_ex", "mmf_gemm_select_impl", "mmf_gemm_last_impl", "mmf_gemm_set_persistent_workgroups",
+    "mmf_gemm7_set_tile_n", "mmf_gemm7_last_tile_n", "mmf_gemm7_tile_n",
     "mmf_attn_fwd_grouped_ex", "mmf_attn_bwd_grouped_ex", "mmf_dropout", "mmf_attn_select_impl",
     "mmf_attn_fwd_grouped", "mmf_attn_bwd_grouped", "mmf_layernorm_fwd_grouped",
     "mmf_layernorm_bwd_grouped", "mmf_layernorm_bwd_workspace_bytes", "mmf_layernorm_last_form", "mmf_cast_f32_to_bf16", "mmf_cast_bf16_to_f32", "mmf_cast_bf16_to_f32_scaled", "mmf_cast_f32_to_bf16_2d", "mmf_add3_bf16", "mmf_add3_grouped", "mmf_addn_bf16", "mmf_addn_grouped",
@@ -120,6 +121,7 @@
     vp, i32, i64, f32 = C.c_void_p, C.c_int, C.c_int64, C.c_float
     lib.mmf_gemm_grouped.argtypes = [C.POINTER(GemmProblem), i32, i32, i32, i32, vp]
     lib.mmf_gemm_grouped_ex.argtypes = [C.POINTER(GemmProblem), i32, i32, i32, i32, C.POINTER(GemmExtra), vp]
+    lib.mmf_gemm7_tile_n.argtypes = [C.POINTER(GemmProblem), i32, i32]
     lib.mmf_attn_fwd_grouped_ex.argtypes = [C.POINTER(AttnProblem), i32, i32, f32, f32, vp, C.c_uint32, vp]
     lib.mmf_attn_bwd_grouped_ex.argtypes = [C.POINTER(AttnProblem), i32, i32, f32, f32, vp, C.c_uint32, vp]
     lib.mmf_dropout.argtypes = [vp, vp, i64, i32, f32, vp, C.c_uint32, vp]
```
